# arielmission-space/PAOS

Measured on AMD Instinct MI355X. Metric: wavefronts/sec (4096^2 c128, 20-surface chain) + achieved HBM GB/s, higher is better.
Workload: dtype c128 (f64); 1 GPU; SYN20 20-surface chain (SURVEY 8d: 43 2-D FFTs per wavefront as the reference runs it), 4096x4096 fp64, walked 512-wavelength sweep, 32 wavefronts/GPU/step, PSFs stay in HBM; separable pass programs + ptp identities ([24] passes/wavefront, parity 1e-15..2e-14 vs oracle); grid=4096, batch_per_gpu=32, parallelism=wavefront-sharded x1, transport=none (single process), ranks_seen=1, launcher=none

## Files before the change

include/paos_hip.h:

```cpp
#ifndef PAOS_HIP_H
#define PAOS_HIP_H

#ifdef __cplusplus
extern "C" {
#endif

typedef struct paos_ctx paos_ctx;

enum { PAOS_OK = 0, PAOS_EINVAL = 1, PAOS_EHIP = 2, PAOS_EUNSUPPORTED = 3 };
enum { PAOS_F64 = 0, PAOS_F32 = 1 };
enum { PAOS_SHAPE_ELLIPSE = 0, PAOS_SHAPE_RECT = 1 };
enum { PAOS_KERNEL_PASS_ROWS = 0, PAOS_KERNEL_PASS_COLS = 1, PAOS_KERNEL_PASS_ANY = 2 };
enum { PAOS_PW_SIGN = 1, PAOS_PW_QPHASE_CENTRED = 2, PAOS_PW_QPHASE_NATURAL = 3, PAOS_PW_SCALE = 4,
       PAOS_PW_MASK = 5 };
enum { PAOS_PWF_MUL2PI = 1,
       PAOS_PWF_X_ONLY = 2, PAOS_PWF_Y_ONLY = 4 };
enum { PAOS_MAX_PW = 6 };
enum { PAOS_NORM_SLOTS = 64 };
enum { PAOS_WHAT_FIELD = 0, PAOS_WHAT_AMPLITUDE = 1, PAOS_WHAT_PHASE = 2, PAOS_WHAT_INTENSITY = 3 };

enum { PAOS_PHASE_STRIDE = 5 };
enum { PAOS_APERTURE_STRIDE = 8 };
enum { PAOS_ZERNIKE_HEAD = 8 };

typedef struct { int kind, flags, block; } paos_pw_op;
typedef struct {
  int axis;
  int fft1, fft2;
  int n_pre, n_mid, n_post;
  paos_pw_op pre[PAOS_MAX_PW], mid[PAOS_MAX_PW], post[PAOS_MAX_PW];
} paos_pass;

typedef struct {
  const double* live_rows;
  int rows_stale;
  int final_intensity;
  int* power_ticket;
  const double* live_cols;
} paos_program_opts;

int paos_ctx_create(int device, int n, int batch, int precision, paos_ctx** out);
int paos_ctx_destroy(paos_ctx* ctx);
const char* paos_last_error(const paos_ctx* ctx);
int paos_sync(paos_ctx* ctx);
const char* paos_build_info(void);
const char* paos_source_hash(void);
void* paos_stream(paos_ctx* ctx);

int paos_profile_begin(paos_ctx* ctx, int kernel_kind, int max_launches);
int paos_profile_end(paos_ctx* ctx, int* launches, double* total_ms);
int paos_profile_end_split(paos_ctx* ctx, int* launches, double* total_ms, int* pruned_launches, double* pruned_ms);
int paos_profile_end_launches(paos_ctx* ctx, int capacity, double* ms_out, int* tag_out, int* count);
int paos_profile_planned_bytes(paos_ctx* ctx, int capacity, double* bytes_out, int* count);
int paos_profile_line_transforms(paos_ctx* ctx, int capacity, double* lines_out, int* count);

int paos_fill(paos_ctx* ctx, double re, double im);
int paos_start(paos_ctx* ctx, double re, double im, int shape, const double* aperture, const double* stop);
int paos_start_rows(paos_ctx* ctx, double re, double im, int shape, const double* aperture, const double* stop,
                    const double* write_rows);
int paos_zero_outside_rows(paos_ctx* ctx, const double* live_rows);
int paos_start_box(paos_ctx* ctx, double re, double im, int shape, const double* aperture, const double* stop,
                   const double* write_rows, const double* write_cols);
int paos_zero_outside_box(paos_ctx* ctx, const double* live_rows, const double* live_cols);
int paos_import(paos_ctx* ctx, int item, const void* host_c128);
int paos_export(paos_ctx* ctx, int item, int what, void* host_out);

int paos_psf_keep(paos_ctx* ctx);
int paos_psf_keep_power(paos_ctx* ctx, int* ticket);
int paos_psf_fetch(paos_ctx* ctx, int item, double* host_out);
int paos_host_alloc(unsigned long long bytes, void** out);
int paos_host_free(void* p);
int paos_export_pinned(paos_ctx* ctx, int item, int what, void* pinned_out);

int paos_aperture(paos_ctx* ctx, int shape, const double* params);
int paos_aperture_render(paos_ctx* ctx, int shape, const double* params1, double* host_mask);
int paos_make_stop(paos_ctx* ctx, const double* enable);
int paos_stop_scale_last_power(paos_ctx* ctx, const double* enable);
int paos_stop_defer_last_power(paos_ctx* ctx, const double* enable);
int paos_norm2(paos_ctx* ctx, double* host_out);
int paos_norm2_enqueue(paos_ctx* ctx, int* ticket);
int paos_norm2_enqueue_rows(paos_ctx* ctx, const double* live_rows, int* ticket);
int paos_norm2_enqueue_rows_like(paos_ctx* ctx, const double* live_rows, const double* same_as, int* ticket);
int paos_norm2_enqueue_box(paos_ctx* ctx, const double* live_rows, const double* live_cols, const double* same_as, int* ticket);
int paos_norm2_fetch(paos_ctx* ctx, int ticket, double* host_out);
int paos_norm2_release(paos_ctx* ctx, int ticket);
int paos_psf_metrics(paos_ctx* ctx, int nr, const double* radii_px, double cx_px, double cy_px,
                     double* host_out);
int paos_phase(paos_ctx* ctx, const double* params, int mul2pi);
int paos_phase_map(paos_ctx* ctx, int item, const double* host_wfe, double wl);
int paos_phase_map_items(paos_ctx* ctx, const double* host_wfe, unsigned long long key, int n_items, const double* items,
                         const double* wl);
int paos_psd_screen(paos_ctx* ctx, const double* host_noise, const double* host_rough, const double* params,
                    unsigned long long key, double* host_out);
int paos_ptp(paos_ctx* ctx, const double* params);
int paos_stw(paos_ctx* ctx, const double* params, int inverse);
int paos_wts(paos_ctx* ctx, const double* params, int inverse);
int paos_run_passes(paos_ctx* ctx, const paos_pass* passes, int n_passes, const double* blocks,
                    int n_blocks);
int paos_copy_yardstick(paos_ctx* ctx, int reps, double* ms_per_launch, double* bytes_per_launch);
int paos_record_set_stats(paos_ctx* ctx, unsigned long long* found, unsigned long long* rendered);
int paos_ctx_set_pruning(paos_ctx* ctx, int on);
int paos_run_passes_live(paos_ctx* ctx, const paos_pass* passes, int n_passes, const double* blocks,
                         int n_blocks, const double* live_rows);
int paos_run_program(paos_ctx* ctx, const paos_pass* passes, int n_passes, const double* blocks, int n_blocks,
                     const paos_program_opts* opts);
int paos_zernike(paos_ctx* ctx, int nmax, int kdim, const double* table, const double* params,
                 int param_stride, double* host_wfe);
int paos_zernike_like(paos_ctx* ctx, int nmax, int kdim, const double* table, const double* params,
                      int param_stride, const double* same_as, double* host_wfe);


int paos_pupil_aperture(paos_ctx* ctx, int shape, const double* params);
int paos_pupil_upload(paos_ctx* ctx, int item, const double* host_weights);
int paos_zernike_gram(paos_ctx* ctx, int nmax, int kdim, const double* table, const double* params,
                      int param_stride, int K, const double* poly, int use_pupil, double* host_out);
int paos_zernike_pupil(paos_ctx* ctx, int nmax, int kdim, const double* table, const double* params,
                       int param_stride, double* host_wfe);

enum { PAOS_DETECTOR_GEOM = 6 };
enum { PAOS_DETECTOR_ITEM = 3 };
enum { PAOS_DETECTOR_SCRATCH_MIB = 512 };
int paos_detector_begin(paos_ctx* ctx, const double* geom);
int paos_detector_add(paos_ctx* ctx, const double* per_item);
int paos_detector_images(paos_ctx* ctx, const double* per_item, double* host_out);
int paos_detector_fetch(paos_ctx* ctx, double* host_out);
enum { PAOS_DETECTOR_PLACED_ITEM = 5 };
int paos_detector_add_placed(paos_ctx* ctx, const double* per_item);
int paos_detector_images_placed(paos_ctx* ctx, const double* per_item, double* host_out);

#ifdef __cplusplus
}
#endif
#endif
```

paos_amd/_lib.py:

```python
import ctypes
import os
import threading
import weakref

import numpy as np

_HERE = os.path.dirname(os.path.abspath(__file__))
LIB_PATH = os.environ.get("PAOS_LIB") or os.path.join(_HERE, "libpaoship.so")

PAOS_F64, PAOS_F32 = 0, 1
SHAPE_ELLIPSE, SHAPE_RECT = 0, 1
WHAT_FIELD, WHAT_AMPLITUDE, WHAT_PHASE, WHAT_INTENSITY = 0, 1, 2, 3
KERNEL_PASS_ROWS, KERNEL_PASS_COLS, KERNEL_PASS_ANY = 0, 1, 2
PW_SIGN, PW_QPHASE_CENTRED, PW_QPHASE_NATURAL, PW_SCALE, PW_MASK = 1, 2, 3, 4, 5
PWF_MUL2PI = 1
PWF_X_ONLY, PWF_Y_ONLY = 2, 4
MAX_PW = 6
NORM_SLOTS = 64


class PwOp(ctypes.Structure):
    _fields_ = [("kind", ctypes.c_int), ("flags", ctypes.c_int), ("block", ctypes.c_int)]


class ProgramOpts(ctypes.Structure):
    _fields_ = [("live_rows", ctypes.POINTER(ctypes.c_double)), ("rows_stale", ctypes.c_int),
                ("final_intensity", ctypes.c_int), ("power_ticket", ctypes.POINTER(ctypes.c_int)),
                ("live_cols", ctypes.POINTER(ctypes.c_double))]


class Pass(ctypes.Structure):
    _fields_ = [("axis", ctypes.c_int), ("fft1", ctypes.c_int), ("fft2", ctypes.c_int),
                ("n_pre", ctypes.c_int), ("n_mid", ctypes.c_int), ("n_post", ctypes.c_int),
                ("pre", PwOp * MAX_PW), ("mid", PwOp * MAX_PW), ("post", PwOp * MAX_PW)]

PHASE_STRIDE = 5
APERTURE_STRIDE = 8
ZERNIKE_HEAD = 8

_c_ctx = ctypes.c_void_p
_dbl_p = ctypes.POINTER(ctypes.c_double)
SYMBOLS = {
    "paos_ctx_create": (ctypes.c_int, [ctypes.c_int, ctypes.c_int, ctypes.c_int, ctypes.c_int, ctypes.POINTER(_c_ctx)]),
    "paos_ctx_destroy": (ctypes.c_int, [_c_ctx]),
    "paos_last_error": (ctypes.c_char_p, [_c_ctx]),
    "paos_sync": (ctypes.c_int, [_c_ctx]),
    "paos_build_info": (ctypes.c_char_p, []),
    "paos_stream": (ctypes.c_void_p, [_c_ctx]),
    "paos_profile_begin": (ctypes.c_int, [_c_ctx, ctypes.c_int, ctypes.c_int]),
    "paos_profile_end": (ctypes.c_int, [_c_ctx, ctypes.POINTER(ctypes.c_int), _dbl_p]),
    "paos_profile_end_split": (ctypes.c_int, [_c_ctx, ctypes.POINTER(ctypes.c_int), _dbl_p, ctypes.POINTER(ctypes.c_int), _dbl_p]),
    "paos_source_hash": (ctypes.c_char_p, []),
    "paos_profile_planned_bytes": (ctypes.c_int, [_c_ctx, ctypes.c_int, _dbl_p, ctypes.POINTER(ctypes.c_int)]),
    "paos_profile_line_transforms": (ctypes.c_int, [_c_ctx, ctypes.c_int, _dbl_p, ctypes.POINTER(ctypes.c_int)]),
    "paos_profile_end_launches": (ctypes.c_int, [_c_ctx, ctypes.c_int, _dbl_p, ctypes.POINTER(ctypes.c_int),
                                                 ctypes.POINTER(ctypes.c_int)]),
    "paos_fill": (ctypes.c_int, [_c_ctx, ctypes.c_double, ctypes.c_double]),
    "paos_import": (ctypes.c_int, [_c_ctx, ctypes.c_int, ctypes.c_void_p]),
    "paos_export": (ctypes.c_int, [_c_ctx, ctypes.c_int, ctypes.c_int, ctypes.c_void_p]),
    "paos_aperture": (ctypes.c_int, [_c_ctx, ctypes.c_int, _dbl_p]),
    "paos_aperture_render": (ctypes.c_int, [_c_ctx, ctypes.c_int, _dbl_p, _dbl_p]),
    "paos_make_stop": (ctypes.c_int, [_c_ctx, _dbl_p]),
    "paos_stop_scale_last_power": (ctypes.c_int, [_c_ctx, _dbl_p]),
    "paos_stop_defer_last_power": (ctypes.c_int, [_c_ctx, _dbl_p]),
    "paos_norm2": (ctypes.c_int, [_c_ctx, _dbl_p]),
    "paos_norm2_enqueue": (ctypes.c_int, [_c_ctx, ctypes.POINTER(ctypes.c_int)]),
    "paos_norm2_fetch": (ctypes.c_int, [_c_ctx, ctypes.c_int, _dbl_p]),
    "paos_norm2_release": (ctypes.c_int, [_c_ctx, ctypes.c_int]),
    "paos_psf_metrics": (ctypes.c_int, [_c_ctx, ctypes.c_int, _dbl_p, ctypes.c_double, ctypes.c_double, _dbl_p]),
    "paos_phase": (ctypes.c_int, [_c_ctx, _dbl_p, ctypes.c_int]),
    "paos_phase_map": (ctypes.c_int, [_c_ctx, ctypes.c_int, _dbl_p, ctypes.c_double]),
    "paos_ptp": (ctypes.c_int, [_c_ctx, _dbl_p]),
    "paos_stw": (ctypes.c_int, [_c_ctx, _dbl_p, ctypes.c_int]),
    "paos_wts": (ctypes.c_int, [_c_ctx, _dbl_p, ctypes.c_int]),
    "paos_run_passes": (ctypes.c_int, [_c_ctx, ctypes.POINTER(Pass), ctypes.c_int, _dbl_p, ctypes.c_int]),
    "paos_copy_yardstick": (ctypes.c_int, [_c_ctx, ctypes.c_int, _dbl_p, _dbl_p]),
    "paos_record_set_stats": (ctypes.c_int, [_c_ctx, ctypes.POINTER(ctypes.c_ulonglong), ctypes.POINTER(ctypes.c_ulonglong)]),
    "paos_ctx_set_pruning": (ctypes.c_int, [_c_ctx, ctypes.c_int]),
    "paos_run_passes_live": (ctypes.c_int, [_c_ctx, ctypes.POINTER(Pass), ctypes.c_int, _dbl_p, ctypes.c_int, _dbl_p]),
    "paos_zernike": (ctypes.c_int, [_c_ctx, ctypes.c_int, ctypes.c_int, _dbl_p, _dbl_p, ctypes.c_int, _dbl_p]),
    "paos_psf_keep": (ctypes.c_int, [_c_ctx]),
    "paos_psf_keep_power": (ctypes.c_int, [_c_ctx, ctypes.POINTER(ctypes.c_int)]),
    "paos_psf_fetch": (ctypes.c_int, [_c_ctx, ctypes.c_int, _dbl_p]),
    "paos_host_alloc": (ctypes.c_int, [ctypes.c_ulonglong, ctypes.POINTER(ctypes.c_void_p)]),
    "paos_host_free": (ctypes.c_int, [ctypes.c_void_p]),
    "paos_export_pinned": (ctypes.c_int, [_c_ctx, ctypes.c_int, ctypes.c_int, ctypes.c_void_p]),
    "paos_start": (ctypes.c_int, [_c_ctx, ctypes.c_double, ctypes.c_double, ctypes.c_int, _dbl_p, _dbl_p]),
    "paos_pupil_aperture": (ctypes.c_int, [_c_ctx, ctypes.c_int, _dbl_p]),
    "paos_pupil_upload": (ctypes.c_int, [_c_ctx, ctypes.c_int, _dbl_p]),
    "paos_zernike_like": (ctypes.c_int, [_c_ctx, ctypes.c_int, ctypes.c_int, _dbl_p, _dbl_p, ctypes.c_int, _dbl_p, _dbl_p]),
    "paos_zernike_gram": (ctypes.c_int, [_c_ctx, ctypes.c_int, ctypes.c_int, _dbl_p, _dbl_p, ctypes.c_int,
                                         ctypes.c_int, _dbl_p, ctypes.c_int, _dbl_p]),
    "paos_zernike_pupil": (ctypes.c_int, [_c_ctx, ctypes.c_int, ctypes.c_int, _dbl_p, _dbl_p, ctypes.c_int, _dbl_p]),
    "paos_start_rows": (ctypes.c_int, [_c_ctx, ctypes.c_double, ctypes.c_double, ctypes.c_int, _dbl_p, _dbl_p, _dbl_p]),
    "paos_zero_outside_rows": (ctypes.c_int, [_c_ctx, _dbl_p]),
    "paos_phase_map_items": (ctypes.c_int, [_c_ctx, _dbl_p, ctypes.c_ulonglong, ctypes.c_int, _dbl_p, _dbl_p]),
    "paos_psd_screen": (ctypes.c_int, [_c_ctx, _dbl_p, _dbl_p, _dbl_p, ctypes.c_ulonglong, _dbl_p]),
    "paos_start_box": (ctypes.c_int, [_c_ctx, ctypes.c_double, ctypes.c_double, ctypes.c_int, _dbl_p, _dbl_p, _dbl_p, _dbl_p]),
    "paos_zero_outside_box": (ctypes.c_int, [_c_ctx, _dbl_p, _dbl_p]),
    "paos_norm2_enqueue_box": (ctypes.c_int, [_c_ctx, _dbl_p, _dbl_p, _dbl_p, ctypes.POINTER(ctypes.c_int)]),
    "paos_norm2_enqueue_rows": (ctypes.c_int, [_c_ctx, _dbl_p, ctypes.POINTER(ctypes.c_int)]),
    "paos_norm2_enqueue_rows_like": (ctypes.c_int, [_c_ctx, _dbl_p, _dbl_p, ctypes.POINTER(ctypes.c_int)]),
    "paos_run_program": (ctypes.c_int, [_c_ctx, ctypes.POINTER(Pass), ctypes.c_int, _dbl_p, ctypes.c_int,
                                        ctypes.POINTER(ProgramOpts)]),
    "paos_detector_begin": (ctypes.c_int, [_c_ctx, _dbl_p]),
    "paos_detector_add": (ctypes.c_int, [_c_ctx, _dbl_p]),
    "paos_detector_images": (ctypes.c_int, [_c_ctx, _dbl_p, _dbl_p]),
    "paos_detector_fetch": (ctypes.c_int, [_c_ctx, _dbl_p]),
    "paos_detector_add_placed": (ctypes.c_int, [_c_ctx, _dbl_p]),
    "paos_detector_images_placed": (ctypes.c_int, [_c_ctx, _dbl_p, _dbl_p]),
}

_lib = None


class PaosHipError(RuntimeError):
    pass


def load():
    global _lib
    if _lib is not None:
        return _lib
    if not os.path.exists(LIB_PATH):
        raise PaosHipError(
            f"{LIB_PATH} not found: build it with `make` or "
            "`python -c 'import __graft_entry__ as g; g.build()'` (there is no CPU fallback)"
        )
    lib = ctypes.CDLL(LIB_PATH)
    if os.environ.get("PAOS_LIB"):
        import sys

        print(f"paos_amd: using the library variant {LIB_PATH} (PAOS_LIB)", file=sys.stderr)
    for name, (res, args) in SYMBOLS.items():
        fn = getattr(lib, name)
        fn.restype = res
        fn.argtypes = args
    _lib = lib
    return lib


def _dptr(arr):
    return arr.ctypes.data_as(_dbl_p)


def as_blocks(blocks, batch, stride):
    arr = np.ascontiguousarray(blocks, dtype=np.float64)
    if arr.shape != (batch, stride):
        raise ValueError(f"expected parameter blocks of shape {(batch, stride)}, got {arr.shape}")
    return arr


PINNED_MIN_BYTES = 4 << 20
PINNED_MAX_BYTES = 32 << 20
PINNED_LIVE_BYTES = int(os.environ.get("PAOS_PINNED_BYTES", 8 << 30))
PINNED_POOL_BYTES = 2 << 30
_pin_lock = threading.Lock()
_pin_free = {}
_pin_live = 0
_pin_pooled = 0
# ... 293 lines not shown

    def norm2_release(self, ticket):
        if hasattr(ticket, "release"):
            return ticket.release()
        self._check(self._lib.paos_norm2_release(self._ctx, int(ticket)), "paos_norm2_release")

    def psf_metrics(self, radii_px=(), centre=None):
        r = np.ascontiguousarray(radii_px, dtype=np.float64).reshape(-1)
        cxp, cyp = (self.n / 2, self.n / 2) if centre is None else centre
        out = np.empty((self.batch, 4 + r.size), dtype=np.float64)
        self._check(self._lib.paos_psf_metrics(self._ctx, int(r.size), _dptr(r) if r.size else None,
                                               float(cxp), float(cyp), _dptr(out)), "paos_psf_metrics")
        res = []
        for row in out:
            p = row[0]
            res.append({"power": p, "centroid": (row[1] / p, row[2] / p) if p > 0 else (np.nan, np.nan),
                        "peak": row[3], "encircled": row[4:].copy()})
        return res

    def phase(self, blocks, mul2pi):
        b = as_blocks(blocks, self.batch, PHASE_STRIDE)
        self._check(self._lib.paos_phase(self._ctx, _dptr(b), int(bool(mul2pi))), "paos_phase")

    def phase_map(self, item, wfe, wl):
        w = np.ascontiguousarray(wfe, dtype=np.float64)
        if w.shape != (self.n, self.n):
            raise ValueError(f"phase map must have shape {(self.n, self.n)}")
        self._check(self._lib.paos_phase_map(self._ctx, int(item), _dptr(w), float(wl)), "paos_phase_map")

    def phase_map_items(self, wfe, items, wls, key=0):
        w = None
        if wfe is not None:
            w = np.ascontiguousarray(wfe, dtype=np.float64)
            if w.shape != (self.n, self.n):
                raise ValueError(f"phase map must have shape {(self.n, self.n)}")
        it = np.ascontiguousarray(items, dtype=np.float64).reshape(-1)
        wl = np.ascontiguousarray(wls, dtype=np.float64).reshape(-1)
        if it.size != wl.size or it.size < 1:
            raise ValueError("one wavelength per listed item is required")
        self._check(self._lib.paos_phase_map_items(self._ctx, _dptr(w) if w is not None else None, int(key) & 0xFFFFFFFFFFFFFFFF,
                                                   int(it.size), _dptr(it), _dptr(wl)), "paos_phase_map_items")

    def psd_screen(self, noise, rough, params, key, want_map=False):
        nz = np.ascontiguousarray(noise, dtype=np.float64)
        if nz.shape != (self.n, self.n):
            raise ValueError(f"the noise must have shape {(self.n, self.n)}")
        rg = None
        if rough is not None:
            rg = np.ascontiguousarray(rough, dtype=np.float64)
            if rg.shape != (self.n, self.n):
                raise ValueError(f"the roughness draw must have shape {(self.n, self.n)}")
        pr = np.ascontiguousarray(params, dtype=np.float64).reshape(-1)
        if pr.size != 12:
            raise ValueError("twelve PSD parameters are required")
        out = np.empty((self.n, self.n), dtype=np.float64) if want_map else None
        self._check(self._lib.paos_psd_screen(self._ctx, _dptr(nz), _dptr(rg) if rg is not None else None, _dptr(pr),
                                              int(key) & 0xFFFFFFFFFFFFFFFF, _dptr(out) if out is not None else None), "paos_psd_screen")
        return out

    def ptp(self, blocks):
        b = as_blocks(blocks, self.batch, PHASE_STRIDE)
        self._check(self._lib.paos_ptp(self._ctx, _dptr(b)), "paos_ptp")

    def stw(self, blocks, inverse):
        b = as_blocks(blocks, self.batch, PHASE_STRIDE)
        self._check(self._lib.paos_stw(self._ctx, _dptr(b), int(bool(inverse))), "paos_stw")

    def wts(self, blocks, inverse):
        b = as_blocks(blocks, self.batch, PHASE_STRIDE)
        self._check(self._lib.paos_wts(self._ctx, _dptr(b), int(bool(inverse))), "paos_wts")

    def copy_yardstick(self, reps=10):
        ms, nbytes = ctypes.c_double(0.0), ctypes.c_double(0.0)
        self._check(self._lib.paos_copy_yardstick(self._ctx, int(reps), ctypes.byref(ms), ctypes.byref(nbytes)),
                    "paos_copy_yardstick")
        return ms.value, nbytes.value

    def record_set_stats(self):
        found, rendered = ctypes.c_ulonglong(0), ctypes.c_ulonglong(0)
        self._check(self._lib.paos_record_set_stats(self._ctx, ctypes.byref(found), ctypes.byref(rendered)),
                    "paos_record_set_stats")
        return int(found.value), int(rendered.value)

    def set_pruning(self, on):
        self._check(self._lib.paos_ctx_set_pruning(self._ctx, 1 if on else 0), "paos_ctx_set_pruning")

    def run_passes(self, passes, blocks, live_rows=None, rows_stale=False, final_intensity=False, live_cols=None):
        b = np.ascontiguousarray(blocks, dtype=np.float64)
        if b.ndim != 3 or b.shape[1:] != (self.batch, PHASE_STRIDE):
            raise ValueError("blocks must be [n_blocks][batch][5]")
        arr = (Pass * len(passes))()
        for dst, src in zip(arr, passes):
            dst.axis, dst.fft1, dst.fft2 = src["axis"], src.get("fft1", -1), src.get("fft2", -1)
            for name in ("pre", "mid", "post"):
                ops = src.get(name, ())
                if len(ops) > MAX_PW:
                    raise ValueError("too many operators in one pass slot")
                setattr(dst, "n_" + name, len(ops))
                lst = getattr(dst, name)
                for i, (kind, flags, block) in enumerate(ops):
                    lst[i].kind, lst[i].flags, lst[i].block = kind, flags, block
        if rows_stale or final_intensity:
            lr = self._rows(live_rows) if live_rows is not None else None
            lc = self._rows(live_cols) if (live_cols is not None and rows_stale and lr is not None) else None
            ticket = ctypes.c_int(-1)
            opts = ProgramOpts(_dptr(lr) if lr is not None else None, 1 if (rows_stale and lr is not None) else 0,
                               int(final_intensity), ctypes.pointer(ticket), _dptr(lc) if lc is not None else None)
            self._check(self._lib.paos_run_program(self._ctx, arr, len(passes), _dptr(b), b.shape[0], ctypes.byref(opts)),
                        "paos_run_program")
            return ticket.value if final_intensity else None
        if live_rows is not None:
            lr = self._rows(live_rows)
            self._check(self._lib.paos_run_passes_live(self._ctx, arr, len(passes), _dptr(b), b.shape[0], _dptr(lr)),
                        "paos_run_passes_live")
            return None
        self._check(self._lib.paos_run_passes(self._ctx, arr, len(passes), _dptr(b), b.shape[0]),
                    "paos_run_passes")
        return None

    def zernike(self, nmax, kdim, table, blocks, want_wfe=False, pupil=False, same_as=None):
        t = np.ascontiguousarray(table, dtype=np.float64).reshape(-1)
        b = np.ascontiguousarray(blocks, dtype=np.float64)
        if b.ndim != 2 or b.shape[0] != self.batch:
            raise ValueError("zernike blocks must be [batch][stride]")
        out = np.empty((self.n, self.n), dtype=np.float64) if want_wfe else None
        if same_as is not None and not pupil:
            like = np.ascontiguousarray(same_as, dtype=np.float64).reshape(-1)
            if like.size != self.batch:
                raise ValueError("same_as must name an item per item")
            self._check(self._lib.paos_zernike_like(self._ctx, int(nmax), int(kdim), _dptr(t), _dptr(b), int(b.shape[1]),
                                                    _dptr(like), _dptr(out) if want_wfe else None), "paos_zernike_like")
            return out
        fn = self._lib.paos_zernike_pupil if pupil else self._lib.paos_zernike
        self._check(fn(self._ctx, int(nmax), int(kdim), _dptr(t), _dptr(b), int(b.shape[1]),
                       _dptr(out) if want_wfe else None),
                    "paos_zernike_pupil" if pupil else "paos_zernike")
        return out

    def start(self, value, shape, blocks, stop=None, write_rows=None, write_cols=None):
        b = np.ascontiguousarray(blocks, dtype=np.float64)
        if b.shape != (self.batch, APERTURE_STRIDE):
            raise ValueError("aperture blocks must be [batch][8]")
        st = None if stop is None else np.ascontiguousarray(stop, dtype=np.float64)
        if st is not None and st.shape != (self.batch,):
            raise ValueError("stop flags must be [batch]")
        v = complex(value)
        if write_rows is not None and write_cols is not None:
            self._check(self._lib.paos_start_box(self._ctx, v.real, v.imag, int(shape), _dptr(b),
                                                 _dptr(st) if st is not None else None, _dptr(self._rows(write_rows)),
                                                 _dptr(self._rows(write_cols))), "paos_start_box")
            return
        if write_rows is not None:
            self._check(self._lib.paos_start_rows(self._ctx, v.real, v.imag, int(shape), _dptr(b),
                                                  _dptr(st) if st is not None else None, _dptr(self._rows(write_rows))),
                        "paos_start_rows")
            return
        self._check(self._lib.paos_start(self._ctx, v.real, v.imag, int(shape), _dptr(b),
                                         _dptr(st) if st is not None else None), "paos_start")

    def pupil_aperture(self, shape, blocks):
        b = np.ascontiguousarray(blocks, dtype=np.float64)
        if b.shape != (self.batch, APERTURE_STRIDE):
            raise ValueError("aperture blocks must be [batch][8]")
        self._check(self._lib.paos_pupil_aperture(self._ctx, int(shape), _dptr(b)), "paos_pupil_aperture")

    def pupil_upload(self, item, weights):
# ... 20 lines not shown
```

paos_amd/csrc/paos_hip.hip:

```cpp
#ifndef PAOS_PART
#define PAOS_PART -1
#endif
#include "../../include/paos_hip.h"

#include <hip/hip_runtime.h>

#include <cmath>
#include <complex>
#include <cstdio>
#include <cstdlib>
#include <cstring>
#include <mutex>
#include <set>
#include <string>
#include <utility>
#include <type_traits>
#include <vector>

#include "frugal_pass.h"
#if PAOS_PART <= 0
#include "pointwise.h"
#endif

using namespace paos;

#ifndef PAOS_BR
#define PAOS_BR 4
#endif
#ifndef PAOS_PAD_BLOCKS
#define PAOS_PAD_BLOCKS 3
#endif
static constexpr int BR = PAOS_BR;
#ifndef PAOS_F32_BR
#define PAOS_F32_BR 8
#endif
template <typename T, int N>
constexpr int block_rows() { return (sizeof(T) == 4 && N >= 2048) ? PAOS_F32_BR : PAOS_BR; }
#define F32_BR_SWITCH(c, ...)                                                            \
  do {                                                                                   \
    if ((c)->br == PAOS_F32_BR) { constexpr int FBR = PAOS_F32_BR; __VA_ARGS__; }        \
    else { constexpr int FBR = PAOS_BR; __VA_ARGS__; }                                   \
  } while (0)
[[maybe_unused]] static constexpr int kNormSlots = PAOS_NORM_SLOTS;
template <typename T>
struct Lay {
  static constexpr int BC = 2;
};

namespace {

thread_local std::string g_err;

constexpr int kArenaSlabs = 4;
struct Arena {
  double* host = nullptr;
  double* dev = nullptr;
  size_t cap = 0, head = 0;
  int cur = 0;
  int left = -1;
  hipEvent_t fence[kArenaSlabs] = {};
  bool fenced[kArenaSlabs] = {};
  bool used[kArenaSlabs] = {};
};

}

struct paos_ctx {
  int device = 0, n = 0, batch = 0, precision = 0;
  int br = PAOS_BR;
  unsigned pitch = 0, item_stride = 0;
  hipStream_t stream = nullptr;
  double* psf = nullptr;
  double* map_dev = nullptr;
  unsigned long long map_key = 0;
  std::vector<double> start_key;
  double* start_norm2 = nullptr;
  cx<double>* psd_scratch = nullptr;
  int* psd_bad = nullptr;
  double* psf_partial = nullptr;
  int psf_nparts = 0;
  double* pow_partial = nullptr;
  int pow_nparts = 0;
  cx<double>* ptab = nullptr;
  int ptab_slots = 0;
  double* dyn_scale = nullptr;
  bool dyn_pending = false;
  bool norm2_of_field = false;
  int psf_zero_axis = -1;
  std::vector<double> psf_zero_lo, psf_zero_hi;
  bool det_set = false;
  int det_nx = 0, det_ny = 0;
  double det_geom[4] = {};
  double* det_img = nullptr;
  double* det_rows = nullptr;
  size_t det_rows_bytes = 0;
  double* det_out = nullptr;
  size_t det_out_bytes = 0;
  void* bounce[2] = {nullptr, nullptr};
  hipEvent_t bounce_ev[2] = {nullptr, nullptr};
  void* field = nullptr;
  void* tw = nullptr;
  void* staging = nullptr;
  cx<double>* tables = nullptr;
  double* mask = nullptr;
  double* metric_partial = nullptr;
  double* metric_out = nullptr;
  double* metric_host = nullptr;
  struct MaskSet {
    MaskLine* lines = nullptr;
    double* vals = nullptr;
    std::vector<double> key;
    unsigned long long used = 0;
    int line_lo = 0, line_hi = 0;
  };
  static constexpr int kMaskSets = 8;
  MaskSet mask_sets[kMaskSets];
  unsigned long long mask_clock = 0;
  unsigned long long mask_hits = 0, mask_rendered = 0;
  size_t lds_pad = 0;
  int* mask_overflow = nullptr;
  double* partial = nullptr;
  double* norm2 = nullptr;
  double* norm2_host = nullptr;
  bool prune = true;
  int norm_slot = 0;
  bool norm_busy[64] = {};
  int nparts = 0;
  Arena arena;
  std::string err;
  int prof_kind = -1;
  std::vector<hipEvent_t> prof_events;
  std::vector<int> prof_tags;
  int prof_next_tag = 0;
  double prof_next_bytes = 0.0;
  std::vector<double> prof_bytes;
  double prof_next_lines = 0.0;
  std::vector<double> prof_lines;
  size_t prof_used = 0;
};

namespace {

int fail(paos_ctx* c, int code, const std::string& msg) {
  if (c) c->err = msg;
  g_err = msg;
  return code;
}

#define HIPCHK(c, call)                                                                     \
  do {                                                                                      \
    hipError_t e_ = (call);                                                                 \
    if (e_ != hipSuccess)                                                                   \
      return fail((c), PAOS_EHIP,                                                           \
                  std::string(#call) + ": " + hipGetErrorString(e_) + " (" __FILE__ ":" +   \
                      std::to_string(__LINE__) + ")");                                      \
  } while (0)

size_t elem_bytes(const paos_ctx* c) { return c->precision == PAOS_F64 ? 16 : 8; }

int arena_switch(paos_ctx* c) {
  Arena& a = c->arena;
  if (a.left >= 0) {
    HIPCHK(c, hipEventRecord(a.fence[a.left], c->stream));
    a.fenced[a.left] = true;
  }
  a.left = a.cur;
  const int next = (a.cur + 1) % kArenaSlabs;
  if (a.used[next]) {
    if (a.fenced[next]) HIPCHK(c, hipEventSynchronize(a.fence[next]));
    else HIPCHK(c, hipStreamSynchronize(c->stream));
  }
  a.fenced[next] = false;
  a.used[next] = true;
  a.cur = next;
  a.head = 0;
  return PAOS_OK;
}

int arena_reserve(paos_ctx* c, size_t total) {
  Arena& a = c->arena;
  total += 64;
  if (total > a.cap) {
    HIPCHK(c, hipStreamSynchronize(c->stream));
    size_t cap = a.cap;
    while (cap < total) cap *= 2;
    double *h = nullptr, *d = nullptr;
    HIPCHK(c, hipHostMalloc(&h, kArenaSlabs * cap * sizeof(double)));
    if (hipMalloc(&d, kArenaSlabs * cap * sizeof(double)) != hipSuccess) {
      (void)hipHostFree(h);
      return fail(c, PAOS_EHIP, "hipMalloc(arena growth)");
    }
    (void)hipHostFree(a.host);
    (void)hipFree(a.dev);
    a.host = h; a.dev = d; a.cap = cap; a.head = 0; a.cur = 0; a.left = -1;
    for (int k = 0; k < kArenaSlabs; ++k) a.fenced[k] = a.used[k] = false;
    a.used[0] = true;
    return PAOS_OK;
  }
  if (a.head + total > a.cap) return arena_switch(c);
  return PAOS_OK;
}

int arena_push(paos_ctx* c, const double* src, size_t count, const double** dev) {
  Arena& a = c->arena;
  if (count > a.cap) return fail(c, PAOS_EINVAL, "parameter block larger than the arena");
  if (a.head + count > a.cap) {
    int rc = arena_switch(c);
    if (rc) return rc;
  }
  double* h = a.host + (size_t)a.cur * a.cap + a.head;
  double* d = a.dev + (size_t)a.cur * a.cap + a.head;
  std::memcpy(h, src, count * sizeof(double));
  HIPCHK(c, hipMemcpyAsync(d, h, count * sizeof(double), hipMemcpyHostToDevice, c->stream));
  *dev = d;
  a.head += (count + 15) & ~size_t(15);
  return PAOS_OK;
}

constexpr size_t kBounceBytes = size_t(4) << 20;
int copy_to_host(paos_ctx* c, void* host, const void* dev, size_t bytes) {
  if (bytes > kBounceBytes) {
    HIPCHK(c, hipMemcpyAsync(host, dev, bytes, hipMemcpyDeviceToHost, c->stream));
    HIPCHK(c, hipStreamSynchronize(c->stream));
    return PAOS_OK;
  }
  for (int i = 0; i < 2; ++i)
    if (!c->bounce[i]) {
      HIPCHK(c, hipHostMalloc(&c->bounce[i], kBounceBytes));
      HIPCHK(c, hipEventCreateWithFlags(&c->bounce_ev[i], hipEventDisableTiming));
    }
  const size_t chunks = (bytes + kBounceBytes - 1) / kBounceBytes;
  auto len = [&](size_t k) { return k + 1 < chunks ? kBounceBytes : bytes - k * kBounceBytes; };
  for (size_t k = 0; k <= chunks; ++k) {
    if (k < chunks) {
      HIPCHK(c, hipMemcpyAsync(c->bounce[k & 1], (const char*)dev + k * kBounceBytes, len(k), hipMemcpyDeviceToHost, c->stream));
      HIPCHK(c, hipEventRecord(c->bounce_ev[k & 1], c->stream));
    }
    if (k > 0) {
      HIPCHK(c, hipEventSynchronize(c->bounce_ev[(k - 1) & 1]));
      std::memcpy((char*)host + (k - 1) * kBounceBytes, c->bounce[(k - 1) & 1], len(k - 1));
    }
  }
  HIPCHK(c, hipStreamSynchronize(c->stream));
  return PAOS_OK;
}

#if PAOS_PART <= 0
int pw_blocks(const paos_ctx* c) {
  const size_t total = (size_t)c->item_stride;
  size_t b = (total + kPwThreads - 1) / kPwThreads;
  return (int)(b < 2048 ? b : 2048);
}
#endif

template <typename T, int N>
struct FftCfg {
  static constexpr int BC = Lay<T>::BC;
  static constexpr int BR = block_rows<T, N>();
  static constexpr int E = 16;
  static constexpr int ROW_LINES = (N >= 2048) ? PAOS_BR / 2 : PAOS_BR;
  static constexpr int FR_ROW_LINES = (N >= 2048) ? BR / 2 : BR;
  static constexpr int COL_LINES = BC;
  static constexpr int ROW_THREADS = ROW_LINES * N / E, COL_THREADS = COL_LINES * N / E;
  static constexpr int ROW_TILES = (ROW_THREADS >= 128) ? 1 : 128 / ROW_THREADS;
  static constexpr int COL_TILES = (COL_THREADS >= 128) ? 1 : 128 / COL_THREADS;
  static constexpr bool ROW_SPLIT = (size_t)ROW_LINES * ROW_TILES * line_lds_bytes<T, N, false>() > 144 * 1024;
  static constexpr bool COL_SPLIT = (size_t)COL_LINES * COL_TILES * line_lds_bytes<T, N, false>() > 144 * 1024;
  static constexpr int MINW = 1;
};

bool timed_launch_begin(paos_ctx* c, int kind) {
  const bool timed = (c->prof_kind == kind || c->prof_kind == PAOS_KERNEL_PASS_ANY) && (c->prof_used + 2 <= c->prof_events.size());
  return timed && hipEventRecord(c->prof_events[c->prof_used], c->stream) == hipSuccess;
}
hipError_t timed_launch_end(paos_ctx* c, int tag) {
  const hipError_t e = hipEventRecord(c->prof_events[c->prof_used + 1], c->stream);
  if (e != hipSuccess) return e;
// ... 411 lines not shown
  }
}
template <typename T, int N, int AXIS>
int frugal_kpre(paos_ctx* c, const FrugalArgs& a, int kpre, int kmid, int nfft) {
  switch (kpre) {
    case 0: return frugal_kmid<T, N, AXIS, 0>(c, a, kmid, nfft);
    case 1: return frugal_kmid<T, N, AXIS, 1>(c, a, kmid, nfft);
    default: return frugal_kmid<T, N, AXIS, 2>(c, a, kmid, nfft);
  }
}
template <typename T, int N>
int frugal_axis(paos_ctx* c, const FrugalArgs& a, int axis, int kpre, int kmid, int nfft) {
  return axis == 0 ? frugal_kpre<T, N, 0>(c, a, kpre, kmid, nfft) : frugal_kpre<T, N, 1>(c, a, kpre, kmid, nfft);
}

}

#define PAOS_HIDDEN __attribute__((visibility("hidden")))
PAOS_HIDDEN int paos_frugal_d1024(paos_ctx* c, const FrugalArgs& a, int axis, int kpre, int kmid, int nfft);
PAOS_HIDDEN int paos_frugal_d2048(paos_ctx* c, const FrugalArgs& a, int axis, int kpre, int kmid, int nfft);
PAOS_HIDDEN int paos_frugal_d4096(paos_ctx* c, const FrugalArgs& a, int axis, int kpre, int kmid, int nfft);
PAOS_HIDDEN int paos_frugal_f2048(paos_ctx* c, const FrugalArgs& a, int axis, int kpre, int kmid, int nfft);
PAOS_HIDDEN int paos_frugal_f4096(paos_ctx* c, const FrugalArgs& a, int axis, int kpre, int kmid, int nfft);
#if PAOS_PART < 0 || PAOS_PART == 1
int paos_frugal_d1024(paos_ctx* c, const FrugalArgs& a, int axis, int kpre, int kmid, int nfft) {
  return frugal_axis<double, 1024>(c, a, axis, kpre, kmid, nfft);
}
#endif
#if PAOS_PART < 0 || PAOS_PART == 2
int paos_frugal_d2048(paos_ctx* c, const FrugalArgs& a, int axis, int kpre, int kmid, int nfft) {
  return frugal_axis<double, 2048>(c, a, axis, kpre, kmid, nfft);
}
#endif
#if PAOS_PART < 0 || PAOS_PART == 3
int paos_frugal_d4096(paos_ctx* c, const FrugalArgs& a, int axis, int kpre, int kmid, int nfft) {
  return frugal_axis<double, 4096>(c, a, axis, kpre, kmid, nfft);
}
#endif
#if PAOS_PART < 0 || PAOS_PART == 4
int paos_frugal_f2048(paos_ctx* c, const FrugalArgs& a, int axis, int kpre, int kmid, int nfft) {
  return frugal_axis<float, 2048>(c, a, axis, kpre, kmid, nfft);
}
#endif
#if PAOS_PART < 0 || PAOS_PART == 5
int paos_frugal_f4096(paos_ctx* c, const FrugalArgs& a, int axis, int kpre, int kmid, int nfft) {
  return frugal_axis<float, 4096>(c, a, axis, kpre, kmid, nfft);
}
#endif

#if PAOS_PART <= 0
namespace {

__global__ void dyn_scale_set_kernel(double* dyn, const double* norm2, const double* enable, int batch) {
  const int i = blockIdx.x * blockDim.x + threadIdx.x;
  if (i < batch) dyn[i] = (!enable || enable[i] != 0.0) ? 1.0 / sqrt(norm2[i]) : 1.0;
}
__global__ void dyn_scale_reset_kernel(double* dyn, int batch) {
  const int i = blockIdx.x * blockDim.x + threadIdx.x;
  if (i < batch) dyn[i] = 1.0;
}
template <typename T>
__global__ void scale_by_kernel(cx<T>* field, const double* dyn, unsigned item_stride) {
  const int item = blockIdx.y;
  const double s = dyn[item];
  if (s == 1.0) return;
  cx<T>* f = field + (size_t)item * item_stride;
  for (size_t m = (size_t)blockIdx.x * blockDim.x + threadIdx.x; m < item_stride; m += (size_t)gridDim.x * blockDim.x)
    f[m] = {(T)__dmul_rn((double)f[m].x, s), (T)__dmul_rn((double)f[m].y, s)};
}
int settle_scale(paos_ctx* c, bool field_is_overwritten = false) {
  if (!c->dyn_pending) return PAOS_OK;
  if (!field_is_overwritten) {
    const dim3 grid(pw_blocks(c), c->batch), block(kPwThreads);
    if (c->precision == PAOS_F64)
      hipLaunchKernelGGL(scale_by_kernel<double>, grid, block, 0, c->stream, (cx<double>*)c->field, c->dyn_scale, c->item_stride);
    else
      hipLaunchKernelGGL(scale_by_kernel<float>, grid, block, 0, c->stream, (cx<float>*)c->field, c->dyn_scale, c->item_stride);
  }
  hipLaunchKernelGGL(dyn_scale_reset_kernel, dim3((c->batch + 255) / 256), dim3(256), 0, c->stream, c->dyn_scale, c->batch);
  HIPCHK(c, hipGetLastError());
  c->dyn_pending = false;
  return PAOS_OK;
}
#define SETTLE_SCALE(c) do { if (c) { (c)->norm2_of_field = false; if ((c)->dyn_pending) { int rc_ = settle_scale(c); if (rc_) return rc_; } } } while (0)
#define DROP_SCALE(c) do { if (c) { (c)->norm2_of_field = false; if ((c)->dyn_pending) { int rc_ = settle_scale(c, true); if (rc_) return rc_; } } } while (0)


bool frugal_sizes(const paos_ctx* c) {
  return use_frugal() && c->n >= (c->precision == PAOS_F64 ? 1024 : 2048);
}

int ensure_mask_store(paos_ctx* c) {
  if (!c->mask_overflow) {
    HIPCHK(c, hipMalloc(&c->mask_overflow, sizeof(int)));
    HIPCHK(c, hipMemsetAsync(c->mask_overflow, 0, sizeof(int), c->stream));
  }
  return PAOS_OK;
}

int mask_render_mode() {
  const char* e = getenv("PAOS_MASK_SCAN");
  if (e && e[0] == '1') return 0;
  const char* pe = getenv("PAOS_MASK_PAIRS");
  return (pe && pe[0] == '0') ? 1 : ((pe && pe[0] == '1') ? 2 : 3);
}
bool mask_rect_blocks() {
  const char* e = getenv("PAOS_MASK_RECT_BLOCKS");
  return !(e && e[0] == '0');
}

int assign_mask_set(paos_ctx* c, const paos_pass& p, LoweredPass& lp, const double* blocks) {
  std::vector<double> key;
  key.reserve((size_t)2 * c->batch * FP_STRIDE + c->batch + 3);
  key.push_back((double)p.axis);
  key.push_back((double)(mask_render_mode() + (mask_rect_blocks() ? 0 : 8)));
  const double* ap = blocks + (size_t)lp.mask_block * c->batch * FP_STRIDE;
  key.insert(key.end(), ap, ap + (size_t)2 * c->batch * FP_STRIDE);
  key.insert(key.end(), lp.mask_shared.begin(), lp.mask_shared.end());
  int hit = -1, victim = 0;
  for (int k = 0; k < paos_ctx::kMaskSets; ++k) {
    const paos_ctx::MaskSet& ms = c->mask_sets[k];
    if (!ms.key.empty() && ms.key.size() == key.size() && !std::memcmp(ms.key.data(), key.data(), key.size() * sizeof(double))) hit = k;
    if (ms.used < c->mask_sets[victim].used) victim = k;
  }
  const int k = hit >= 0 ? hit : victim;
  paos_ctx::MaskSet& ms = c->mask_sets[k];
  if (!ms.lines) {
    for (paos_ctx::MaskSet& m2 : c->mask_sets) {
      if (m2.lines) continue;
      HIPCHK(c, hipMalloc(&m2.lines, (size_t)c->batch * c->n * sizeof(MaskLine)));
      HIPCHK(c, hipMalloc(&m2.vals, (size_t)c->batch * c->n * 2 * kMaskW * sizeof(double)));
    }
  }
  ms.used = ++c->mask_clock;
  lp.mask_set = k;
  lp.mask_render = hit < 0;
  lp.mask_shapes = 0;
  for (int it = 0; it < c->batch; ++it) {
    const double* a1 = ap + (size_t)it * FP_STRIDE;
    const double* a2 = a1 + (size_t)c->batch * FP_STRIDE;
    if (a1[0] != 0.0 && (it >= (int)lp.mask_shared.size() || lp.mask_shared[it] == 0.0)) lp.mask_shapes |= (int)a2[3] == 0 ? 1 : 2;
  }
  if (hit < 0) { ms.key = std::move(key); ++c->mask_rendered; } else ++c->mask_hits;
  for (int it = 0; it < c->batch; ++it) {
    if (lp.mask_rep[it] < 0) continue;
    FrugalSlot& sl = lp.mask_slot == 0 ? lp.items[it].pre : lp.items[it].mid;
    sl.lines = ms.lines + (size_t)lp.mask_rep[it] * c->n;
    sl.vals = ms.vals + (size_t)lp.mask_rep[it] * c->n * 2 * kMaskW;
  }
  return PAOS_OK;
}

void forget_mask_sets(paos_ctx* c) {
  for (auto& ms : c->mask_sets) ms.key.clear();
}

MaskJob mask_job(paos_ctx* c, const paos_pass& p, const LoweredPass& lp, const double* ap, const double* dshared) {
  const paos_ctx::MaskSet& ms = c->mask_sets[lp.mask_set];
  const int line0 = lp.mask_lo, line_end = lp.mask_hi > lp.mask_lo ? lp.mask_hi : c->n;
  return MaskJob{ap, dshared, ms.lines, ms.vals, p.axis, line0, line_end, lp.mask_shapes};
}
int launch_mask_jobs(paos_ctx* c, MaskJobs& jobs, int count) {
  jobs.batch_stride = c->batch * (int)FP_STRIDE; jobs.param_stride = (int)FP_STRIDE; jobs.n = c->n; jobs.overflow = c->mask_overflow;
  {
    const int mode = mask_render_mode();
    jobs.windows = mode != 0 ? 1 : 0;
    jobs.pairs = mode >= 2 ? mode - 1 : 0;
    jobs.rect_blocks = mask_rect_blocks() ? 1 : 0;
// ... 216 lines not shown
  int rc;
  if ((rc = check_ops(c, p.pre, p.n_pre, n_blocks))) return rc;
  if ((rc = check_ops(c, p.mid, p.n_mid, n_blocks))) return rc;
  if ((rc = check_ops(c, p.post, p.n_post, n_blocks))) return rc;
  if (p.fft1 >= n_blocks || p.fft2 >= n_blocks) return fail(c, PAOS_EINVAL, "transform control block out of range");
  {
    const paos_pw_op* lists3[3] = {p.pre, p.mid, p.post};
    const int counts3[3] = {p.n_pre, p.n_mid, p.n_post};
    int nmask = 0;
    for (int l = 0; l < 3; ++l)
      for (int o = 0; o < counts3[l]; ++o)
        if (lists3[l][o].kind == PAOS_PW_MASK) {
          if (++nmask > 1) return fail(c, PAOS_EINVAL, "one aperture operator per pass");
          if (!c->mask) HIPCHK(c, hipMalloc(&c->mask, (size_t)c->batch * c->item_stride * sizeof(double)));
          const double* ap = dblocks + (size_t)lists3[l][o].block * c->batch * FP_STRIDE;
          const dim3 grid(pw_blocks(c), c->batch), block(kPwThreads);
          const double* ap2 = ap + (size_t)c->batch * FP_STRIDE;
          if (c->precision == PAOS_F64) {
            hipLaunchKernelGGL((aperture_kernel<double, BR, Lay<double>::BC, 0>), grid, block, 0, c->stream, (cx<double>*)nullptr, ap, ap2, FP_STRIDE, c->n, c->pitch, c->item_stride, c->mask, 1);
            hipLaunchKernelGGL((aperture_kernel<double, BR, Lay<double>::BC, 1>), grid, block, 0, c->stream, (cx<double>*)nullptr, ap, ap2, FP_STRIDE, c->n, c->pitch, c->item_stride, c->mask, 1);
          } else {
            F32_BR_SWITCH(c, hipLaunchKernelGGL((aperture_kernel<float, FBR, Lay<float>::BC, 0>), grid, block, 0, c->stream, (cx<float>*)nullptr, ap, ap2, FP_STRIDE, c->n, c->pitch, c->item_stride, c->mask, 1));
            F32_BR_SWITCH(c, hipLaunchKernelGGL((aperture_kernel<float, FBR, Lay<float>::BC, 1>), grid, block, 0, c->stream, (cx<float>*)nullptr, ap, ap2, FP_STRIDE, c->n, c->pitch, c->item_stride, c->mask, 1));
          }
          HIPCHK(c, hipGetLastError());
        }
  }
  PassArgs a{};
  a.field = c->field; a.tw = c->tw; a.blocks = dblocks; a.tables = c->tables; a.mask = c->mask; a.batch = c->batch;
  a.fft1 = p.fft1; a.fft2 = p.fft2; a.n_pre = p.n_pre; a.n_mid = p.n_mid; a.n_post = p.n_post;
  static_assert(sizeof(PwOp) == sizeof(paos_pw_op), "ABI op layout");
  std::memcpy(a.pre, p.pre, sizeof(a.pre));
  std::memcpy(a.mid, p.mid, sizeof(a.mid));
  std::memcpy(a.post, p.post, sizeof(a.post));
  PwOp* lists[3] = {a.pre, a.mid, a.post};
  const int counts[3] = {a.n_pre, a.n_mid, a.n_post};
  int feat = 0;
  for (int l = 0; l < 3; ++l)
    for (int o = 0; o < PAOS_MAX_PW; ++o) {
      lists[l][o].flags &= (1 << kTableShift) - 1;
      const int t = table_of_op[l * PAOS_MAX_PW + o];
      if (t >= 0) { lists[l][o].flags |= (t + 1) << kTableShift; feat = 3; }
      if (o < counts[l] && lists[l][o].kind == PWK_MASK) feat = 3;
    }
  a.pitch = c->pitch; a.item_stride = c->item_stride;
  if (p.axis == 0 || p.axis == 1)
    return c->precision == PAOS_F64 ? pass_t<double>(c, p.axis, a, feat) : pass_t<float>(c, p.axis, a, feat);
  if (p.axis != -1) return fail(c, PAOS_EINVAL, "pass axis must be 0, 1 or -1");
  if (p.fft1 >= 0 || p.fft2 >= 0 || p.n_mid || p.n_post)
    return fail(c, PAOS_EINVAL, "a transform-free pass carries its operators in the pre list");
  const dim3 grid(pw_blocks(c), c->batch), block(kPwThreads);
  if (c->precision == PAOS_F64)
    hipLaunchKernelGGL((pointwise_kernel<double, BR, Lay<double>::BC>), grid, block, 0, c->stream, a, c->n);
  else
    F32_BR_SWITCH(c, hipLaunchKernelGGL((pointwise_kernel<float, FBR, Lay<float>::BC>), grid, block, 0, c->stream, a, c->n));
  HIPCHK(c, hipGetLastError());
  return PAOS_OK;
}

bool use_pruning() {
  static const bool on = [] { const char* e = getenv("PAOS_NO_PRUNE"); return !(e && e[0] == '1'); }();
  return on;
}

int zero_outside_rows(paos_ctx* c, const double* live_rows);
int zero_outside_box(paos_ctx* c, const double* live_rows, const double* live_cols);
int psf_power_ticket(paos_ctx* c, const double* partial, int nparts, int* ticket, const double* source = nullptr);
int psf_keep_power_impl(paos_ctx* c, int* ticket);

int run_passes_impl(paos_ctx* c, const paos_pass* passes, int n_passes, const double* blocks, int n_blocks,
                    const double* entry_rows, bool entry_stale, int* final_ticket, int final_mode, const double* entry_cols);

int run_passes(paos_ctx* c, const paos_pass* passes, int n_passes, const double* blocks, int n_blocks,
               const double* entry_rows = nullptr, bool entry_stale = false, int* final_ticket = nullptr, int final_mode = 1,
               const double* entry_cols = nullptr) {
  const int rc = run_passes_impl(c, passes, n_passes, blocks, n_blocks, entry_rows, entry_stale, final_ticket, final_mode, entry_cols);
  if (rc != PAOS_OK && c) forget_mask_sets(c);
  return rc;
}

int run_passes_impl(paos_ctx* c, const paos_pass* passes, int n_passes, const double* blocks, int n_blocks,
                    const double* entry_rows, bool entry_stale, int* final_ticket, int final_mode, const double* entry_cols) {
  if (!c || !passes || !blocks || n_passes < 0 || n_blocks < 1) return fail(c, PAOS_EINVAL, "bad pass program");
  c->norm2_of_field = false;
  if (final_ticket && c->norm_busy[next_norm_slot(c)])
    return fail(c, PAOS_EINVAL, "64 power reductions outstanding: fetch earlier tickets (paos_norm2_fetch) first");
  for (int i = 0; i < n_passes; ++i) {
    const paos_pw_op* lists[3] = {passes[i].pre, passes[i].mid, passes[i].post};
    const int counts[3] = {passes[i].n_pre, passes[i].n_mid, passes[i].n_post};
    for (int l = 0; l < 3; ++l)
      for (int o = 0; o < counts[l] && o < PAOS_MAX_PW; ++o) {
        const paos_pw_op& op = lists[l][o];
        if (op.kind != PAOS_PW_QPHASE_CENTRED && op.kind != PAOS_PW_QPHASE_NATURAL) continue;
        if (op.block < 0 || op.block >= n_blocks) return fail(c, PAOS_EINVAL, "operator block index out of range");
        for (int it = 0; it < c->batch; ++it) {
          const double* p = blocks + ((size_t)op.block * c->batch + it) * FP_STRIDE;
          if (p[FP_ENABLE] == 0.0) continue;
          const double hx = 0.5 * c->n * p[FP_SX], hy = 0.5 * c->n * p[FP_SY];
          double arg = std::fabs(p[FP_COEF]) * (hx * hx + hy * hy);
          if (op.flags & PAOS_PWF_MUL2PI) arg *= 6.283185307179586;
          if (!(arg < kMaxPhaseArg))
            return fail(c, PAOS_EUNSUPPORTED, "quadratic phase exceeds 1e12 rad at the grid corner (or is not finite)");
        }
      }
  }
  const double* dblocks = nullptr;
  const size_t per_pass = (((size_t)c->batch * sizeof(FrugalItem) / sizeof(double) + 15) & ~size_t(15)) +
                          (((size_t)c->batch + 15) & ~size_t(15)) + 16;
  int rc = arena_reserve(c, (size_t)n_blocks * c->batch * FP_STRIDE + 16 + (size_t)n_passes * per_pass);
  if (rc) return rc;
  rc = arena_push(c, blocks, (size_t)n_blocks * c->batch * FP_STRIDE, &dblocks);
  if (rc) return rc;
  std::vector<LoweredPass> low(n_passes);
  bool all_frugal = !use_tables() && frugal_sizes(c) && n_passes > 0;
  if (!use_tables() && frugal_sizes(c)) {
    if ((rc = ensure_mask_store(c))) return rc;
    for (int q = 0; q < n_passes; ++q) {
      LoweredPass& lp = low[q];
      lp.ok = lower_frugal(c, passes[q], blocks, lp.items, lp.kpre, lp.kmid, lp.nfft, lp.mask_block, lp.mask_slot, lp.mask_shared,
                           lp.mask_rep);
      if (lp.ok && lp.mask_block >= 0 && (rc = assign_mask_set(c, passes[q], lp, blocks))) return rc;
      all_frugal = all_frugal && lp.ok;
    }
  }
  if (c->dyn_pending) {
    bool ride = n_passes > 0 && low[0].ok;
    if (ride)
      for (const FrugalItem& fi : low[0].items) ride = ride && fi.active != 0.0;
    if (!ride && (rc = settle_scale(c))) return rc;
  }
  const bool pruned = all_frugal && use_pruning() && c->prune;
  if (pruned) plan_pruning(c, passes, n_passes, blocks, low, entry_rows, entry_stale, entry_cols);
  {
    for (int q = 0; q < n_passes; ++q) {
      LoweredPass& lp = low[q];
      if (!lp.ok || lp.mask_block < 0) continue;
      double lo = (double)c->n, hi = 0.0;
      for (const FrugalItem& fi : lp.items) {
        if (fi.active == 0.0) continue;
        lo = fi.line_lo < lo ? fi.line_lo : lo;
        hi = fi.line_hi > hi ? fi.line_hi : hi;
      }
      const bool window = hi > lo;
      lp.mask_lo = window ? (int)lo : 0;
      lp.mask_hi = window ? (int)hi : c->n;
      paos_ctx::MaskSet& ms = c->mask_sets[lp.mask_set];
      if (!lp.mask_render && !(ms.line_lo <= lp.mask_lo && ms.line_hi >= lp.mask_hi)) {
        lp.mask_render = true;
        --c->mask_hits; ++c->mask_rendered;
      }
      if (lp.mask_render) { ms.line_lo = lp.mask_lo; ms.line_hi = lp.mask_hi; }
    }
  }
  if (entry_stale && entry_rows) {
    bool need = !pruned;
    for (int it = 0; it < c->batch && !need; ++it) {
      bool active = false;
      for (int q = 0; q < n_passes; ++q) active = active || low[q].items[it].active != 0.0;
      need = !active;
    }
    const double* windows[2] = {entry_rows, entry_cols};
    for (int w = 0; w < 2 && !need; ++w)
      for (int it = 0; windows[w] && it < c->batch && !need; ++it) {
        const int br = c->br, l = ((int)windows[w][2 * it] / br) * br;
        int h = (((int)windows[w][2 * it + 1] + br - 1) / br) * br;
        if (h > c->n) h = c->n;
// ... 435 lines not shown
  }
  if (c->arena.host) (void)hipHostFree(c->arena.host);
  if (c->arena.dev) (void)hipFree(c->arena.dev);
  for (int k = 0; k < kArenaSlabs; ++k)
    if (c->arena.fence[k]) (void)hipEventDestroy(c->arena.fence[k]);
  if (c->stream) (void)hipStreamDestroy(c->stream);
  delete c;
  return PAOS_OK;
}

static int check_mask_overflow(paos_ctx* c) {
  if (!c->mask_overflow) return PAOS_OK;
  int n = 0;
  HIPCHK(c, hipMemcpy(&n, c->mask_overflow, sizeof(int), hipMemcpyDeviceToHost));
  if (n != 0) {
    (void)hipMemset(c->mask_overflow, 0, sizeof(int));
    for (auto& ms : c->mask_sets) ms.key.clear();
    return fail(c, PAOS_EUNSUPPORTED, "aperture line records overflowed (partial run longer than kMaskW): results are invalid");
  }
  return PAOS_OK;
}

int paos_sync(paos_ctx* c) {
  if (c) (void)hipSetDevice(c->device);
  if (!c) return fail(c, PAOS_EINVAL, "null context");
  HIPCHK(c, hipStreamSynchronize(c->stream));
  return check_mask_overflow(c);
}

int paos_fill(paos_ctx* c, double re, double im) {
  DROP_SCALE(c);
  if (c) (void)hipSetDevice(c->device);
  if (!c) return fail(c, PAOS_EINVAL, "null context");
  const size_t total = (size_t)c->item_stride * c->batch;
  if (c->precision == PAOS_F64)
    hipLaunchKernelGGL(fill_kernel<double>, dim3(2048), dim3(kPwThreads), 0, c->stream,
                       (cx<double>*)c->field, total, re, im);
  else
    hipLaunchKernelGGL(fill_kernel<float>, dim3(2048), dim3(kPwThreads), 0, c->stream,
                       (cx<float>*)c->field, total, (float)re, (float)im);
  HIPCHK(c, hipGetLastError());
  return PAOS_OK;
}

static int check_rows(paos_ctx* c, const double* rows) {
  for (int i = 0; i < c->batch; ++i)
    if (!(rows[2 * i] >= 0.0) || !(rows[2 * i + 1] <= (double)c->n) || !(rows[2 * i] <= rows[2 * i + 1]))
      return fail(c, PAOS_EINVAL, "row range must satisfy 0 <= lo <= hi <= n");
  return PAOS_OK;
}

static std::vector<double> rounded_cols(const paos_ctx* c, const double* cols) {
  std::vector<double> out((size_t)2 * c->batch);
  for (int i = 0; i < c->batch; ++i) {
    int l = (int)cols[2 * i], h = (int)cols[2 * i + 1];
    l = l < 0 ? 0 : (l / c->br) * c->br;
    h = ((h + c->br - 1) / c->br) * c->br;
    if (h > c->n) h = c->n;
    out[2 * i] = l; out[2 * i + 1] = h;
  }
  return out;
}

static int start_impl(paos_ctx* c, double re, double im, int shape, const double* aperture, const double* stop,
                      const double* write_rows, const double* write_cols = nullptr) {
  if (c) (void)hipSetDevice(c->device);
  if (!c || !aperture) return fail(c, PAOS_EINVAL, "null argument");
  if (shape != PAOS_SHAPE_ELLIPSE && shape != PAOS_SHAPE_RECT) return fail(c, PAOS_EINVAL, "unknown aperture shape");
  std::vector<double> flags(c->batch, 0.0);
  bool any_stop = false;
  if (stop)
    for (int i = 0; i < c->batch; ++i) { flags[i] = stop[i] != 0.0 ? 1.0 : 0.0; any_stop |= flags[i] != 0.0; }
  std::vector<double> power_of(c->batch), compute(c->batch);
  for (int i = 0; i < c->batch; ++i) {
    int rep = i;
    for (int j = 0; j < i; ++j)
      if (flags[j] != 0.0 && !std::memcmp(aperture + (size_t)j * AP_STRIDE, aperture + (size_t)i * AP_STRIDE, AP_STRIDE * sizeof(double))) { rep = j; break; }
    power_of[i] = (double)rep;
    compute[i] = (flags[i] != 0.0 && rep == i) ? 1.0 : 0.0;
  }
  const double *dp = nullptr, *ds = nullptr, *dcompute = nullptr, *dpower_of = nullptr;
  int rc;
  if ((rc = arena_push(c, aperture, (size_t)c->batch * AP_STRIDE, &dp))) return rc;
  if ((rc = arena_push(c, flags.data(), flags.size(), &ds))) return rc;
  if ((rc = arena_push(c, compute.data(), compute.size(), &dcompute))) return rc;
  if ((rc = arena_push(c, power_of.data(), power_of.size(), &dpower_of))) return rc;
  const double* drows = nullptr;
  if (write_rows) {
    if ((rc = check_rows(c, write_rows))) return rc;
    if ((rc = arena_push(c, write_rows, (size_t)2 * c->batch, &drows))) return rc;
  }
  const double* dcols = nullptr;
  if (write_cols) {
    if (!write_rows) return fail(c, PAOS_EINVAL, "a column window needs a row window");
    if ((rc = check_rows(c, write_cols))) return rc;
    const std::vector<double> wc = rounded_cols(c, write_cols);
    if ((rc = arena_push(c, wc.data(), wc.size(), &dcols))) return rc;
  }
  static const bool share_start = [] { const char* e = getenv("PAOS_SHARE_START"); return !(e && e[0] == '0'); }();
  std::vector<double> goff(c->batch, 0.0), glen(c->batch, 0.0), members;
  {
    std::vector<int> lead(c->batch);
    for (int i = 0; i < c->batch; ++i) {
      lead[i] = i;
      if (!share_start) continue;
      for (int j = 0; j < i; ++j)
        if (lead[j] == j && flags[j] == flags[i] &&
            !std::memcmp(aperture + (size_t)j * AP_STRIDE, aperture + (size_t)i * AP_STRIDE, AP_STRIDE * sizeof(double)) &&
            (!write_rows || !std::memcmp(write_rows + 2 * j, write_rows + 2 * i, 2 * sizeof(double))) &&
            (!write_cols || !std::memcmp(write_cols + 2 * j, write_cols + 2 * i, 2 * sizeof(double)))) { lead[i] = j; break; }
    }
    for (int i = 0; i < c->batch; ++i) {
      if (lead[i] != i) continue;
      goff[i] = (double)members.size();
      for (int j = i; j < c->batch; ++j)
        if (lead[j] == i) members.push_back((double)j);
      glen[i] = (double)members.size() - goff[i];
    }
  }
  const double *dgoff = nullptr, *dglen = nullptr, *dmembers = nullptr;
  if ((rc = arena_push(c, goff.data(), goff.size(), &dgoff))) return rc;
  if ((rc = arena_push(c, glen.data(), glen.size(), &dglen))) return rc;
  if ((rc = arena_push(c, members.data(), members.size(), &dmembers))) return rc;
  const dim3 block(kPwThreads);
  bool power_found = false;
  if (any_stop) {
    static const bool memo = [] { const char* e = getenv("PAOS_START_POWER_MEMO"); return !(e && e[0] == '0'); }();
    std::vector<double> key;
    key.reserve(3 + (size_t)c->batch * (AP_STRIDE + 1));
    key.push_back((double)shape); key.push_back(re); key.push_back(im);
    key.insert(key.end(), aperture, aperture + (size_t)c->batch * AP_STRIDE);
    key.insert(key.end(), flags.begin(), flags.end());
    power_found = memo && c->start_norm2 && key.size() == c->start_key.size() &&
                  !std::memcmp(key.data(), c->start_key.data(), key.size() * sizeof(double));
    if (power_found) {
      HIPCHK(c, hipMemcpyAsync(c->norm2, c->start_norm2, (size_t)c->batch * sizeof(double), hipMemcpyDeviceToDevice, c->stream));
    } else {
      c->start_key.clear();
      if (memo) c->start_key = std::move(key);
    }
  }
#define START_LAUNCH(T, BRV, S)                                                                         \
  do {                                                                                                  \
    if (any_stop && !power_found) {                                                                     \
      hipLaunchKernelGGL((start_power_kernel<T, BRV, Lay<T>::BC, S>), dim3(c->nparts, c->batch), block, 0, \
                         c->stream, dp, c->n, c->pitch, c->item_stride, re, im, c->partial, dcompute);  \
      hipLaunchKernelGGL(norm2_final_kernel, dim3(c->batch), block, 0, c->stream, c->partial, c->norm2,   \
                         c->nparts, ds, 1, dpower_of);                                                  \
    }                                                                                                   \
    hipLaunchKernelGGL((start_write_kernel<T, BRV, Lay<T>::BC, S>), dim3(pw_blocks(c), c->batch), block, 0, \
                       c->stream, (cx<T>*)c->field, dp, c->n, c->pitch, c->item_stride, re, im,          \
                       (const double*)c->norm2, ds, drows, dgoff, dglen, dmembers, dcols);              \
  } while (0)
  if (c->precision == PAOS_F64) {
    if (shape == PAOS_SHAPE_ELLIPSE) START_LAUNCH(double, BR, 0); else START_LAUNCH(double, BR, 1);
  } else {
    if (shape == PAOS_SHAPE_ELLIPSE) F32_BR_SWITCH(c, START_LAUNCH(float, FBR, 0)); else F32_BR_SWITCH(c, START_LAUNCH(float, FBR, 1));
  }
#undef START_LAUNCH
  HIPCHK(c, hipGetLastError());
  if (any_stop && !power_found && !c->start_key.empty()) {
    if (!c->start_norm2) HIPCHK(c, hipMalloc(&c->start_norm2, (size_t)c->batch * sizeof(double)));
    HIPCHK(c, hipMemcpyAsync(c->start_norm2, c->norm2, (size_t)c->batch * sizeof(double), hipMemcpyDeviceToDevice, c->stream));
  }
  return PAOS_OK;
}

int paos_start(paos_ctx* c, double re, double im, int shape, const double* aperture, const double* stop) {
  DROP_SCALE(c);
  return start_impl(c, re, im, shape, aperture, stop, nullptr);
}

int paos_start_rows(paos_ctx* c, double re, double im, int shape, const double* aperture, const double* stop,
                    const double* write_rows) {
  DROP_SCALE(c);
  return start_impl(c, re, im, shape, aperture, stop, write_rows);
}

int paos_start_box(paos_ctx* c, double re, double im, int shape, const double* aperture, const double* stop,
                   const double* write_rows, const double* write_cols) {
  DROP_SCALE(c);
  return start_impl(c, re, im, shape, aperture, stop, write_rows, write_cols);
}

int paos_zero_outside_box(paos_ctx* c, const double* live_rows, const double* live_cols) {
  SETTLE_SCALE(c);
  if (c) (void)hipSetDevice(c->device);
  if (!c || !live_rows) return fail(c, PAOS_EINVAL, "null argument");
  int rc = check_rows(c, live_rows);
  if (rc) return rc;
  if (live_cols && (rc = check_rows(c, live_cols))) return rc;
  return zero_outside_box(c, live_rows, live_cols);
}

int paos_zero_outside_rows(paos_ctx* c, const double* live_rows) {
  SETTLE_SCALE(c);
  if (c) (void)hipSetDevice(c->device);
  if (!c || !live_rows) return fail(c, PAOS_EINVAL, "null argument");
  int rc = check_rows(c, live_rows);
  if (rc) return rc;
  return zero_outside_rows(c, live_rows);
}

int paos_import(paos_ctx* c, int item, const void* host) {
  SETTLE_SCALE(c);
  if (c) (void)hipSetDevice(c->device);
  if (!c || !host || item < 0 || item >= c->batch) return fail(c, PAOS_EINVAL, "bad item or null buffer");
  const size_t bytes = (size_t)c->n * c->n * 16;
  HIPCHK(c, hipMemcpyAsync(c->staging, host, bytes, hipMemcpyHostToDevice, c->stream));
  if (c->precision == PAOS_F64)
    hipLaunchKernelGGL((import_kernel<double, BR, Lay<double>::BC>), dim3(pw_blocks(c)), dim3(kPwThreads), 0, c->stream,
                       (cx<double>*)c->field + (size_t)item * c->item_stride, (const cx<double>*)c->staging,
                       c->n, c->pitch);
  else
    F32_BR_SWITCH(c, hipLaunchKernelGGL((import_kernel<float, FBR, Lay<float>::BC>), dim3(pw_blocks(c)), dim3(kPwThreads), 0, c->stream,
                       (cx<float>*)c->field + (size_t)item * c->item_stride, (const cx<double>*)c->staging,
                       c->n, c->pitch));
  HIPCHK(c, hipGetLastError());
  HIPCHK(c, hipStreamSynchronize(c->stream));
  return PAOS_OK;
}

static int export_impl(paos_ctx* c, int item, int what, void* host_out, bool pinned) {
  if (!c || !host_out || item < 0 || item >= c->batch || what < 0 || what > 3)
    return fail(c, PAOS_EINVAL, "bad item/what or null buffer");
  if (c->precision == PAOS_F64)
    hipLaunchKernelGGL((export_kernel<double, BR, Lay<double>::BC>), dim3(pw_blocks(c)), dim3(kPwThreads), 0, c->stream,
                       (const cx<double>*)c->field + (size_t)item * c->item_stride, (double*)c->staging,
                       c->n, c->pitch, what);
  else
    F32_BR_SWITCH(c, hipLaunchKernelGGL((export_kernel<float, FBR, Lay<float>::BC>), dim3(pw_blocks(c)), dim3(kPwThreads), 0, c->stream,
                       (const cx<float>*)c->field + (size_t)item * c->item_stride, (double*)c->staging,
                       c->n, c->pitch, what));
  HIPCHK(c, hipGetLastError());
  const size_t bytes = (size_t)c->n * c->n * (what == PAOS_WHAT_FIELD ? 16 : 8);
  if (pinned) {
    HIPCHK(c, hipMemcpyAsync(host_out, c->staging, bytes, hipMemcpyDeviceToHost, c->stream));
    HIPCHK(c, hipStreamSynchronize(c->stream));
  } else {
    int rc = copy_to_host(c, host_out, c->staging, bytes);
    if (rc) return rc;
  }
  return check_mask_overflow(c);
}

int paos_export(paos_ctx* c, int item, int what, void* host_out) {
  SETTLE_SCALE(c);
  if (c) (void)hipSetDevice(c->device);
  return export_impl(c, item, what, host_out, false);
// ... 260 lines not shown
  }
  return PAOS_OK;
}

int zero_outside_box(paos_ctx* c, const double* live_rows, const double* live_cols) {
  if (!live_cols) return zero_outside_rows(c, live_rows);
  const double *drows = nullptr, *dcols = nullptr;
  int rc;
  if ((rc = arena_push(c, live_rows, (size_t)2 * c->batch, &drows))) return rc;
  const std::vector<double> lc = rounded_cols(c, live_cols);
  if ((rc = arena_push(c, lc.data(), lc.size(), &dcols))) return rc;
  const dim3 grid(pw_blocks(c), c->batch), block(kPwThreads);
  if (c->precision == PAOS_F64)
    hipLaunchKernelGGL((zero_outside_box_kernel<double, BR, Lay<double>::BC>), grid, block, 0, c->stream, (cx<double>*)c->field, c->n,
                       c->pitch, c->item_stride, drows, dcols);
  else
    F32_BR_SWITCH(c, hipLaunchKernelGGL((zero_outside_box_kernel<float, FBR, Lay<float>::BC>), grid, block, 0, c->stream,
                                        (cx<float>*)c->field, c->n, c->pitch, c->item_stride, drows, dcols));
  HIPCHK(c, hipGetLastError());
  return PAOS_OK;
}

}

extern "C" {

int paos_psf_keep_power(paos_ctx* c, int* ticket) {
  SETTLE_SCALE(c);
  if (c) (void)hipSetDevice(c->device);
  if (!c || !ticket) return fail(c, PAOS_EINVAL, "null argument");
  return psf_keep_power_impl(c, ticket);
}

int paos_run_program(paos_ctx* c, const paos_pass* passes, int n_passes, const double* blocks, int n_blocks,
                     const paos_program_opts* opts) {
  if (c) (void)hipSetDevice(c->device);
  if (!opts) return run_passes(c, passes, n_passes, blocks, n_blocks);
  if (c && opts->live_rows) {
    int rc = check_rows(c, opts->live_rows);
    if (rc) return rc;
  }
  if (opts->final_intensity && !opts->power_ticket) return fail(c, PAOS_EINVAL, "final_intensity needs a place for the power ticket");
  if (opts->final_intensity < 0 || opts->final_intensity > 2) return fail(c, PAOS_EINVAL, "final_intensity: 0, 1 (PSF instead of the field) or 2 (field + its power)");
  const bool stale = opts->live_rows && opts->rows_stale != 0;
  if (c && opts->live_cols && stale) {
    int rc = check_rows(c, opts->live_cols);
    if (rc) return rc;
  }
  return run_passes(c, passes, n_passes, blocks, n_blocks, opts->live_rows, stale,
                    opts->final_intensity ? opts->power_ticket : nullptr, opts->final_intensity == 2 ? 2 : 1,
                    stale ? opts->live_cols : nullptr);
}

static int norm2_enqueue_rows_impl(paos_ctx* c, const double* live_rows, const double* same_as, int* ticket,
                                   const double* live_cols = nullptr) {
  if (c) (void)hipSetDevice(c->device);
  if (!c || !ticket || !live_rows) return fail(c, PAOS_EINVAL, "null argument");
  int rc = check_rows(c, live_rows);
  if (rc) return rc;
  const int slot = next_norm_slot(c);
  if (c->norm_busy[slot])
    return fail(c, PAOS_EINVAL, "64 power reductions outstanding: fetch earlier tickets (paos_norm2_fetch) first");
  const double *drows = nullptr, *dlead = nullptr, *dsame = nullptr, *dcols = nullptr;
  if ((rc = arena_push(c, live_rows, (size_t)2 * c->batch, &drows))) return rc;
  if (live_cols) {
    const std::vector<double> lc = rounded_cols(c, live_cols);
    if ((rc = arena_push(c, lc.data(), lc.size(), &dcols))) return rc;
  }
  if (same_as) {
    std::vector<double> lead(c->batch);
    for (int i = 0; i < c->batch; ++i) {
      const int j = (int)same_as[i];
      if (!(same_as[i] >= 0.0) || j >= c->batch || (double)j != same_as[i] || (int)same_as[j] != j)
        return fail(c, PAOS_EINVAL, "same_as must name an item that stands for itself");
      if (live_rows[2 * i] != live_rows[2 * j] || live_rows[2 * i + 1] != live_rows[2 * j + 1] ||
          (live_cols && (live_cols[2 * i] != live_cols[2 * j] || live_cols[2 * i + 1] != live_cols[2 * j + 1])))
        return fail(c, PAOS_EINVAL, "items that share a sum must share their row (and column) window");
      lead[i] = j == i ? 1.0 : 0.0;
    }
    if ((rc = arena_push(c, lead.data(), lead.size(), &dlead))) return rc;
    if ((rc = arena_push(c, same_as, (size_t)c->batch, &dsame))) return rc;
  }
  const dim3 grid(c->nparts, c->batch), block(kPwThreads);
  if (c->precision == PAOS_F64)
    hipLaunchKernelGGL((norm2_partial_kernel<double, BR, Lay<double>::BC>), grid, block, 0, c->stream,
                       (const cx<double>*)c->field, c->partial, c->n, c->pitch, c->item_stride, dlead, 1, drows, dcols);
  else
    F32_BR_SWITCH(c, hipLaunchKernelGGL((norm2_partial_kernel<float, FBR, Lay<float>::BC>), grid, block, 0, c->stream,
                       (const cx<float>*)c->field, c->partial, c->n, c->pitch, c->item_stride, dlead, 1, drows, dcols));
  HIPCHK(c, hipGetLastError());
  return psf_power_ticket(c, c->partial, c->nparts, ticket, dsame);
}

int paos_norm2_enqueue_box(paos_ctx* c, const double* live_rows, const double* live_cols, const double* same_as, int* ticket) {
  SETTLE_SCALE(c);
  if (c && live_cols) {
    int rc = check_rows(c, live_cols);
    if (rc) return rc;
  }
  return norm2_enqueue_rows_impl(c, live_rows, same_as, ticket, live_cols);
}

int paos_norm2_enqueue_rows(paos_ctx* c, const double* live_rows, int* ticket) {
  SETTLE_SCALE(c);
  return norm2_enqueue_rows_impl(c, live_rows, nullptr, ticket);
}

int paos_norm2_enqueue_rows_like(paos_ctx* c, const double* live_rows, const double* same_as, int* ticket) {
  SETTLE_SCALE(c);
  if (!same_as) return fail(c, PAOS_EINVAL, "null argument");
  return norm2_enqueue_rows_impl(c, live_rows, same_as, ticket);
}

int paos_norm2_fetch(paos_ctx* c, int ticket, double* host_out) {
  if (c) (void)hipSetDevice(c->device);
  if (!c || !host_out || ticket < 0 || ticket >= kNormSlots) return fail(c, PAOS_EINVAL, "bad ticket");
  if (!c->norm_busy[ticket]) return fail(c, PAOS_EINVAL, "ticket is not outstanding (already fetched, or never issued)");
  HIPCHK(c, hipStreamSynchronize(c->stream));
  c->norm_busy[ticket] = false;
  std::memcpy(host_out, c->norm2_host + (size_t)ticket * c->batch, (size_t)c->batch * sizeof(double));
  return check_mask_overflow(c);
}

int paos_norm2_release(paos_ctx* c, int ticket) {
  if (!c || ticket < 0 || ticket >= kNormSlots) return fail(c, PAOS_EINVAL, "bad ticket");
  c->norm_busy[ticket] = false;
  return PAOS_OK;
}

int paos_norm2(paos_ctx* c, double* host_out) {
  SETTLE_SCALE(c);
  if (c) (void)hipSetDevice(c->device);
  if (!c || !host_out) return fail(c, PAOS_EINVAL, "null argument");
  int rc = norm2_launch(c, nullptr);
  if (rc) return rc;
  HIPCHK(c, hipMemcpyAsync(c->norm2_host, c->norm2, (size_t)c->batch * sizeof(double), hipMemcpyDeviceToHost, c->stream));
  HIPCHK(c, hipStreamSynchronize(c->stream));
  std::memcpy(host_out, c->norm2_host, (size_t)c->batch * sizeof(double));
  return PAOS_OK;
}

int paos_phase(paos_ctx* c, const double* params, int mul2pi) {
  SETTLE_SCALE(c);
  if (c) (void)hipSetDevice(c->device);
  if (!c || !params) return fail(c, PAOS_EINVAL, "null argument");
  Program g(c->batch);
  const int par = g.add_block(params, 0, 0, 0, 0, true);
  paos_pass& p = g.add_pass(-1, -1, -1);
  push(p.pre, p.n_pre, PAOS_PW_QPHASE_CENTRED, par, mul2pi ? PAOS_PWF_MUL2PI : 0);
  return run_passes(c, g.passes.data(), 1, g.blocks.data(), 1);
}

int paos_phase_map(paos_ctx* c, int item, const double* host_wfe, double wl) {
  SETTLE_SCALE(c);
  if (c) (void)hipSetDevice(c->device);
  if (!c || !host_wfe || item < 0 || item >= c->batch) return fail(c, PAOS_EINVAL, "bad item or null buffer");
  if (!(wl > 0.0) || !std::isfinite(wl)) return fail(c, PAOS_EINVAL, "wavelength must be positive and finite");
  const size_t count = (size_t)c->n * c->n;
  for (size_t i = 0; i < count; ++i)
    if (!std::isfinite(host_wfe[i])) return fail(c, PAOS_EINVAL, "the phase map holds a non-finite value (fill masked pixels with 0)");
  HIPCHK(c, hipMemcpyAsync(c->staging, host_wfe, count * sizeof(double), hipMemcpyHostToDevice, c->stream));
  if (c->precision == PAOS_F64)
    hipLaunchKernelGGL((phase_map_kernel<double, BR, Lay<double>::BC>), dim3(pw_blocks(c)), dim3(kPwThreads), 0, c->stream,
                       (cx<double>*)c->field + (size_t)item * c->item_stride, (const double*)c->staging, c->n, c->pitch, wl);
  else
    F32_BR_SWITCH(c, hipLaunchKernelGGL((phase_map_kernel<float, FBR, Lay<float>::BC>), dim3(pw_blocks(c)), dim3(kPwThreads), 0, c->stream,
                       (cx<float>*)c->field + (size_t)item * c->item_stride, (const double*)c->staging, c->n, c->pitch, wl));
  HIPCHK(c, hipGetLastError());
  HIPCHK(c, hipStreamSynchronize(c->stream));
  return PAOS_OK;
}

int paos_phase_map_items(paos_ctx* c, const double* host_wfe, unsigned long long key, int n_items, const double* items,
                         const double* wl) {
  SETTLE_SCALE(c);
  if (c) (void)hipSetDevice(c->device);
  if (!c || !items || !wl || n_items < 1 || n_items > c->batch) return fail(c, PAOS_EINVAL, "bad item list or null buffer");
  if (!host_wfe && (key == 0 || key != c->map_key || !c->map_dev)) return fail(c, PAOS_EINVAL, "no host map, and no map kept on the device under this key");
// ... 9 lines not shown
    c->map_key = 0;
    HIPCHK(c, hipMemcpyAsync(c->map_dev, host_wfe, count * sizeof(double), hipMemcpyHostToDevice, c->stream));
    HIPCHK(c, hipStreamSynchronize(c->stream));
    c->map_key = key;
  }
  const double *ditems = nullptr, *dwl = nullptr;
  int rc;
  if ((rc = arena_push(c, items, (size_t)n_items, &ditems))) return rc;
  if ((rc = arena_push(c, wl, (size_t)n_items, &dwl))) return rc;
  const dim3 grid(pw_blocks(c), n_items), block(kPwThreads);
  if (c->precision == PAOS_F64)
    hipLaunchKernelGGL((phase_map_items_kernel<double, BR, Lay<double>::BC>), grid, block, 0, c->stream, (cx<double>*)c->field,
                       c->item_stride, (const double*)c->map_dev, c->n, c->pitch, ditems, dwl);
  else
    F32_BR_SWITCH(c, hipLaunchKernelGGL((phase_map_items_kernel<float, FBR, Lay<float>::BC>), grid, block, 0, c->stream,
                                        (cx<float>*)c->field, c->item_stride, (const double*)c->map_dev, c->n, c->pitch, ditems, dwl));
  HIPCHK(c, hipGetLastError());
  return PAOS_OK;
}

int paos_psd_screen(paos_ctx* c, const double* host_noise, const double* host_rough, const double* params, unsigned long long key,
                    double* host_out) {
  if (c) (void)hipSetDevice(c->device);
  if (!c || !host_noise || !params || key == 0) return fail(c, PAOS_EINVAL, "null argument (or key 0)");
  if (c->precision != PAOS_F64) return fail(c, PAOS_EUNSUPPORTED, "PSD screens are built on complex128 contexts (build the map on the host for fp32 mode)");
  PsdParams p{params[0], params[1], params[2], params[3], params[4], params[5], params[6], params[7], params[8], params[9], params[10], params[11]};
  for (int k = 0; k < 12; ++k)
    if (std::isnan(params[k])) return fail(c, PAOS_EINVAL, "a PSD parameter is NaN");
  const size_t count = (size_t)c->n * c->n;
  if (!c->map_dev) HIPCHK(c, hipMalloc(&c->map_dev, count * sizeof(double)));
  if (!c->psd_scratch) HIPCHK(c, hipMalloc(&c->psd_scratch, (size_t)c->item_stride * sizeof(cx<double>)));
  if (!c->psd_bad) HIPCHK(c, hipMalloc(&c->psd_bad, sizeof(int)));
  c->map_key = 0;
  double* noise = (double*)c->staging;
  double* rough = (host_rough && p.SR != 0.0) ? noise + count : nullptr;
  HIPCHK(c, hipMemcpyAsync(noise, host_noise, count * sizeof(double), hipMemcpyHostToDevice, c->stream));
  if (rough) HIPCHK(c, hipMemcpyAsync(rough, host_rough, count * sizeof(double), hipMemcpyHostToDevice, c->stream));
  HIPCHK(c, hipMemsetAsync(c->psd_bad, 0, sizeof(int), c->stream));
  std::vector<double> hb((size_t)3 * FP_STRIDE, 0.0);
  hb[0 * FP_STRIDE + FP_ENABLE] = 1.0;
  hb[1 * FP_STRIDE + FP_ENABLE] = 1.0; hb[1 * FP_STRIDE + 1] = 1.0;
  hb[2 * FP_STRIDE + FP_ENABLE] = 1.0; hb[2 * FP_STRIDE + 3] = 1.0 / c->n;
  const double* dblocks = nullptr;
  int rc;
  if ((rc = arena_push(c, hb.data(), hb.size(), &dblocks))) return rc;
  const dim3 grid(pw_blocks(c)), block(kPwThreads);
  hipLaunchKernelGGL((psd_load_kernel<BR, Lay<double>::BC>), grid, block, 0, c->stream, c->psd_scratch, (const double*)noise, c->n, c->pitch);
  PassArgs a{};
  a.field = c->psd_scratch; a.tw = c->tw; a.blocks = dblocks; a.tables = nullptr; a.mask = nullptr; a.batch = 1;
  a.fft1 = 0; a.fft2 = -1; a.pitch = c->pitch; a.item_stride = c->item_stride;
  for (int axis = 0; axis < 2; ++axis)
    if ((rc = pass_t<double>(c, axis, a, 0))) return rc;
  hipLaunchKernelGGL((psd_filter_kernel<BR, Lay<double>::BC>), grid, block, 0, c->stream, c->psd_scratch, c->n, c->pitch, p);
  a.fft1 = 1; a.n_mid = 1; a.mid[0] = {PAOS_PW_SCALE, 0, 2};
  for (int axis = 0; axis < 2; ++axis)
    if ((rc = pass_t<double>(c, axis, a, 0))) return rc;
  hipLaunchKernelGGL((psd_finish_kernel<BR, Lay<double>::BC>), grid, block, 0, c->stream, c->map_dev, (const cx<double>*)c->psd_scratch,
                     (const double*)rough, c->n, c->pitch, p, c->psd_bad);
  HIPCHK(c, hipGetLastError());
  int bad = 0;
  HIPCHK(c, hipMemcpyAsync(&bad, c->psd_bad, sizeof(int), hipMemcpyDeviceToHost, c->stream));
  HIPCHK(c, hipStreamSynchronize(c->stream));
  if (bad) return fail(c, PAOS_EINVAL, "the PSD screen holds a non-finite value");
  if (host_out) {
    rc = copy_to_host(c, host_out, c->map_dev, count * sizeof(double));
    if (rc) return rc;
  }
  c->map_key = key;
  return PAOS_OK;
}

int paos_run_passes(paos_ctx* c, const paos_pass* passes, int n_passes, const double* blocks, int n_blocks) {
  if (c) (void)hipSetDevice(c->device);
  return run_passes(c, passes, n_passes, blocks, n_blocks);
}

int paos_record_set_stats(paos_ctx* c, unsigned long long* found, unsigned long long* rendered) {
  if (!c || !found || !rendered) return fail(c, PAOS_EINVAL, "bad record-set request");
  *found = c->mask_hits;
  *rendered = c->mask_rendered;
  return PAOS_OK;
}

int paos_copy_yardstick(paos_ctx* c, int reps, double* ms_per_launch, double* bytes_per_launch) {
  SETTLE_SCALE(c);
  if (c) (void)hipSetDevice(c->device);
  if (!c || !ms_per_launch || !bytes_per_launch || reps < 1) return fail(c, PAOS_EINVAL, "bad yardstick request");
  const size_t total = (size_t)c->item_stride * c->batch;
  const int blocks = (int)((total + kPwThreads - 1) / kPwThreads < 65536 * 4 ? (total + kPwThreads - 1) / kPwThreads : 65536 * 4);
  hipEvent_t e0, e1;
  HIPCHK(c, hipEventCreate(&e0));
  HIPCHK(c, hipEventCreate(&e1));
  auto launch = [&] {
    if (c->precision == PAOS_F64)
      hipLaunchKernelGGL(rmw_copy_kernel<double>, dim3(blocks), dim3(kPwThreads), 0, c->stream, (cx<double>*)c->field, total);
    else
      hipLaunchKernelGGL(rmw_copy_kernel<float>, dim3(blocks), dim3(kPwThreads), 0, c->stream, (cx<float>*)c->field, total);
  };
  launch();
  HIPCHK(c, hipEventRecord(e0, c->stream));
  for (int r = 0; r < reps; ++r) launch();
  HIPCHK(c, hipEventRecord(e1, c->stream));
  HIPCHK(c, hipEventSynchronize(e1));
  float ms = 0.f;
  HIPCHK(c, hipEventElapsedTime(&ms, e0, e1));
  (void)hipEventDestroy(e0);
  (void)hipEventDestroy(e1);
  *ms_per_launch = (double)ms / reps;
  *bytes_per_launch = 2.0 * (double)total * (double)elem_bytes(c);
  return PAOS_OK;
}

int paos_ctx_set_pruning(paos_ctx* c, int on) {
  if (!c) return fail(c, PAOS_EINVAL, "null context");
  c->prune = on != 0;
  return PAOS_OK;
}

int paos_run_passes_live(paos_ctx* c, const paos_pass* passes, int n_passes, const double* blocks, int n_blocks,
                         const double* live_rows) {
  if (c) (void)hipSetDevice(c->device);
  if (c && live_rows)
    for (int i = 0; i < c->batch; ++i)
      if (!(live_rows[2 * i] >= 0.0) || !(live_rows[2 * i + 1] <= (double)c->n) || !(live_rows[2 * i] <= live_rows[2 * i + 1]))
        return fail(c, PAOS_EINVAL, "live row range must satisfy 0 <= lo <= hi <= n");
  return run_passes(c, passes, n_passes, blocks, n_blocks, live_rows);
}

int paos_ptp(paos_ctx* c, const double* params) {
  if (c) (void)hipSetDevice(c->device);
  return fft_op(c, OP_PTP, params, 0);
}
int paos_stw(paos_ctx* c, const double* params, int inverse) {
  if (c) (void)hipSetDevice(c->device);
  return fft_op(c, OP_STW, params, inverse);
}
int paos_wts(paos_ctx* c, const double* params, int inverse) {
  if (c) (void)hipSetDevice(c->device);
  return fft_op(c, OP_WTS, params, inverse);
}

static int zernike_apply(paos_ctx* c, int nmax, int kdim, const double* table, const double* params,
                         int param_stride, double* host_wfe, bool use_pupil, const double* same_as = nullptr) {
  if (!c || !table || !params) return fail(c, PAOS_EINVAL, "null argument");
  if (nmax < 0 || kdim < nmax / 2 + 1 || param_stride < ZP_HEAD + 2 * (nmax + 1) * kdim)
    return fail(c, PAOS_EINVAL, "inconsistent Zernike table dimensions");
  if (use_pupil && !c->mask) return fail(c, PAOS_EINVAL, "no pupil defined (paos_pupil_aperture / paos_pupil_upload)");
  for (int i = 0; i < c->batch; ++i) {
    const double* q = params + (size_t)i * param_stride;
    if (q[ZP_ENABLE] == 0.0) continue;
    if (!(q[ZP_RADIUS] > 0.0)) return fail(c, PAOS_EINVAL, "Zernike radius must be > 0");
    for (int k = ZP_DX; k < param_stride; ++k)
      if (!std::isfinite(q[k])) return fail(c, PAOS_EINVAL, "non-finite Zernike parameter");
  }
  const double *dt = nullptr, *dp = nullptr;
  int rc = arena_push(c, table, (size_t)(nmax + 1) * kdim * 3, &dt);
  if (rc) return rc;
  rc = arena_push(c, params, (size_t)c->batch * param_stride, &dp);
  if (rc) return rc;
  static const bool share_wfe = [] { const char* e = getenv("PAOS_SHARE_WFE"); return !(e && e[0] == '0'); }();
  std::vector<double> goff(c->batch, 0.0), glen(c->batch, 0.0), members;
  {
    std::vector<int> lead(c->batch, -1);
    auto same_map = [&](int a, int b) {
      const double *qa = params + (size_t)a * param_stride, *qb = params + (size_t)b * param_stride;
      for (int k = 0; k < param_stride; ++k)
        if (k != ZP_INV_WL && std::memcmp(qa + k, qb + k, sizeof(double))) return false;
      return true;
    };
    for (int i = 0; i < c->batch; ++i) {
      if (params[(size_t)i * param_stride + ZP_ENABLE] == 0.0) continue;
      lead[i] = i;
      if (share_wfe && !use_pupil)
        for (int j = 0; j < i; ++j)
          if (lead[j] == j && same_map(j, i)) { lead[i] = j; break; }
    }
    for (int i = 0; i < c->batch; ++i) {
      if (lead[i] != i) continue;
      goff[i] = (double)members.size();
      for (int j = i; j < c->batch; ++j)
        if (lead[j] == i) members.push_back((double)j);
      glen[i] = (double)members.size() - goff[i];
    }
    if (members.empty()) members.push_back(0.0);
  }
  const double *dgoff = nullptr, *dglen = nullptr, *dmembers = nullptr, *dtwins = nullptr;
  if ((rc = arena_push(c, goff.data(), goff.size(), &dgoff))) return rc;
  if ((rc = arena_push(c, glen.data(), glen.size(), &dglen))) return rc;
  if ((rc = arena_push(c, members.data(), members.size(), &dmembers))) return rc;
  if (same_as) {
    std::vector<double> twins(c->batch, 0.0);
    bool any = false;
    for (int i = 0; i < c->batch; ++i) {
      if (!(same_as[i] >= 0.0) || same_as[i] >= (double)c->batch || same_as[i] != (double)(int)same_as[i])
        return fail(c, PAOS_EINVAL, "same_as must hold item indices");
      if (glen[i] < 2.0) continue;
      bool all = true;
      for (int g = 0; g < (int)glen[i]; ++g) all = all && same_as[(int)members[(size_t)goff[i] + g]] == same_as[i];
      twins[i] = all ? 1.0 : 0.0;
      any = any || all;
    }
    if (any && (rc = arena_push(c, twins.data(), twins.size(), &dtwins))) return rc;
  }
  const dim3 grid(pw_blocks(c), c->batch), block(kPwThreads);
  double* wfe = host_wfe ? (double*)c->staging : nullptr;
  const double* pupil = use_pupil ? c->mask : nullptr;
  unsigned m_first = 0, m_end = c->item_stride;
  if (!host_wfe) {
    double half = -1.0;
    bool known = true;
    for (int i = 0; i < c->batch; ++i) {
      const double* q = params + (size_t)i * param_stride;
      if (q[ZP_ENABLE] == 0.0) continue;
      const double h = q[ZP_RADIUS] / q[ZP_DY];
      if (!(h >= 0.0) || !std::isfinite(h)) { known = false; break; }
      if (h > half) half = h;
    }
    if (known && half >= 0.0 && half < (double)c->n) {
      int lo = (int)std::floor((double)(c->n / 2) - half) - 2, hi = (int)std::ceil((double)(c->n / 2) + half) + 3;
      lo = lo < 0 ? 0 : (lo / c->br) * c->br;
      hi = hi > c->n ? c->n : ((hi + c->br - 1) / c->br) * c->br;
      if (hi > c->n) hi = c->n;
      m_first = (unsigned)(lo / c->br) * c->pitch;
      m_end = (unsigned)(hi / c->br) * c->pitch;
    }
  }
#define ZK_LAUNCH(T, BRV, NC)                                                                                          \
  hipLaunchKernelGGL((zernike_kernel<T, BRV, Lay<T>::BC, NC>), grid, block, 0, c->stream, (cx<T>*)c->field, dt, dp,   \
                     param_stride, c->n, c->pitch, c->item_stride, nmax, kdim, wfe, pupil, m_first, m_end, dgoff, dglen, \
                     dmembers, dtwins)
  if (c->precision == PAOS_F64) {
    if (nmax <= 8) ZK_LAUNCH(double, BR, 8); else ZK_LAUNCH(double, BR, 0);
  } else {
    if (nmax <= 8) F32_BR_SWITCH(c, ZK_LAUNCH(float, FBR, 8)); else F32_BR_SWITCH(c, ZK_LAUNCH(float, FBR, 0));
  }
#undef ZK_LAUNCH
  HIPCHK(c, hipGetLastError());
  if (host_wfe) return copy_to_host(c, host_wfe, c->staging, (size_t)c->n * c->n * 8);
  return PAOS_OK;
}

int paos_zernike(paos_ctx* c, int nmax, int kdim, const double* table, const double* params,
                 int param_stride, double* host_wfe) {
  SETTLE_SCALE(c);
  if (c) (void)hipSetDevice(c->device);
  return zernike_apply(c, nmax, kdim, table, params, param_stride, host_wfe, false);
}

int paos_zernike_like(paos_ctx* c, int nmax, int kdim, const double* table, const double* params,
                      int param_stride, const double* same_as, double* host_wfe) {
  SETTLE_SCALE(c);
  if (c) (void)hipSetDevice(c->device);
  return zernike_apply(c, nmax, kdim, table, params, param_stride, host_wfe, false, same_as);
}

int paos_zernike_pupil(paos_ctx* c, int nmax, int kdim, const double* table, const double* params,
                       int param_stride, double* host_wfe) {
  SETTLE_SCALE(c);
  if (c) (void)hipSetDevice(c->device);
  return zernike_apply(c, nmax, kdim, table, params, param_stride, host_wfe, true);
}

static int ensure_pupil(paos_ctx* c) {
  if (!c->mask) HIPCHK(c, hipMalloc(&c->mask, (size_t)c->batch * c->item_stride * sizeof(double)));
  return PAOS_OK;
}

int paos_pupil_aperture(paos_ctx* c, int shape, const double* params) {
  if (c) (void)hipSetDevice(c->device);
  if (!c || !params) return fail(c, PAOS_EINVAL, "null argument");
  if (shape != PAOS_SHAPE_ELLIPSE && shape != PAOS_SHAPE_RECT) return fail(c, PAOS_EINVAL, "unknown aperture shape");
  int rc = ensure_pupil(c);
  if (rc) return rc;
  const double* dp = nullptr;
  rc = arena_push(c, params, (size_t)c->batch * AP_STRIDE, &dp);
  if (rc) return rc;
  const dim3 grid(pw_blocks(c), c->batch), block(kPwThreads);
  if (shape == PAOS_SHAPE_ELLIPSE)
    F32_BR_SWITCH(c, hipLaunchKernelGGL((aperture_kernel<double, FBR, Lay<double>::BC, 0>), grid, block, 0, c->stream, (cx<double>*)nullptr,
                       dp, (const double*)nullptr, AP_STRIDE, c->n, c->pitch, c->item_stride, c->mask, 2));
  else
    F32_BR_SWITCH(c, hipLaunchKernelGGL((aperture_kernel<double, FBR, Lay<double>::BC, 1>), grid, block, 0, c->stream, (cx<double>*)nullptr,
                       dp, (const double*)nullptr, AP_STRIDE, c->n, c->pitch, c->item_stride, c->mask, 2));
  HIPCHK(c, hipGetLastError());
  return PAOS_OK;
}

int paos_pupil_upload(paos_ctx* c, int item, const double* host_weights) {
  if (c) (void)hipSetDevice(c->device);
  if (!c || !host_weights) return fail(c, PAOS_EINVAL, "null argument");
  if (item < 0 || item >= c->batch) return fail(c, PAOS_EINVAL, "item out of range");
  int rc = ensure_pupil(c);
  if (rc) return rc;
  HIPCHK(c, hipMemcpyAsync(c->staging, host_weights, (size_t)c->n * c->n * 8, hipMemcpyHostToDevice, c->stream));
  F32_BR_SWITCH(c, hipLaunchKernelGGL((import_weights_kernel<FBR, Lay<double>::BC>), dim3(pw_blocks(c)), dim3(kPwThreads), 0, c->stream,
                     (const double*)c->staging, c->mask + (size_t)item * c->item_stride, c->n, c->pitch, c->item_stride));
  HIPCHK(c, hipGetLastError());
  HIPCHK(c, hipStreamSynchronize(c->stream));
  return PAOS_OK;
}

int paos_zernike_gram(paos_ctx* c, int nmax, int kdim, const double* table, const double* params,
                      int param_stride, int K, const double* poly, int use_pupil, double* host_out) {
  SETTLE_SCALE(c);
  if (c) (void)hipSetDevice(c->device);
  if (!c || !table || !params || !poly || !host_out) return fail(c, PAOS_EINVAL, "null argument");
  if (nmax < 0 || kdim < nmax / 2 + 1 || param_stride < ZP_HEAD)
    return fail(c, PAOS_EINVAL, "inconsistent Zernike table dimensions");
  if (K < 1 || K > kGramMaxK) return fail(c, PAOS_EUNSUPPORTED, "1 <= K <= 64 polynomials");
  if (use_pupil && !c->mask) return fail(c, PAOS_EINVAL, "no pupil defined (paos_pupil_aperture / paos_pupil_upload)");
  for (int i = 0; i < c->batch; ++i) {
    const double* q = params + (size_t)i * param_stride;
    if (q[ZP_ENABLE] == 0.0) continue;
    if (!(q[ZP_RADIUS] > 0.0)) return fail(c, PAOS_EINVAL, "Zernike radius must be > 0");
    for (int k = ZP_DX; k < ZP_HEAD; ++k)
      if (!std::isfinite(q[k])) return fail(c, PAOS_EINVAL, "non-finite Zernike parameter");
  }
  const size_t ncoef = (size_t)(nmax + 1) * kdim;
  std::vector<double> slots(2 * ncoef, -1.0), fac(K);
  for (int j = 0; j < K; ++j) {
    const int am = (int)poly[4 * j], k = (int)poly[4 * j + 1], is_sin = poly[4 * j + 2] != 0.0;
    if (am < 0 || am > nmax || k < 0 || k >= kdim || am + 2 * k > nmax)
      return fail(c, PAOS_EINVAL, "polynomial outside the recurrence table");
    double& slot = slots[2 * ((size_t)am * kdim + k) + (is_sin ? 1 : 0)];
    if (slot >= 0.0) return fail(c, PAOS_EINVAL, "polynomial listed twice");
    slot = (double)j;
    fac[j] = poly[4 * j + 3];
  }
  const double *dt = nullptr, *dp = nullptr, *dslots = nullptr, *dfac = nullptr;
  int rc;
  if ((rc = arena_push(c, table, ncoef * 3, &dt))) return rc;
  if ((rc = arena_push(c, params, (size_t)c->batch * param_stride, &dp))) return rc;
  if ((rc = arena_push(c, slots.data(), slots.size(), &dslots))) return rc;
  if ((rc = arena_push(c, fac.data(), fac.size(), &dfac))) return rc;
// ... 193 lines not shown
```

paos_amd/csrc/pointwise.h:

```cpp
#pragma once
#include "frugal_pass.h"

namespace paos {

template <int BR, int BC>
__device__ __forceinline__ bool layout_unmap(size_t m, int n, unsigned pitch, int& row, int& col) {
  const unsigned brow = (unsigned)(m / pitch), rem = (unsigned)(m % pitch);
  if (rem >= (unsigned)n * BR) return false;
  const unsigned in = rem % (BR * BC);
  row = (int)(brow * BR + in / BC);
  col = (int)((rem / (BR * BC)) * BC + in % BC);
  return true;
}

constexpr int kPwThreads = 256;

template <typename T>
__global__ void fill_kernel(cx<T>* f, size_t total, T re, T im) {
  size_t i = (size_t)blockIdx.x * blockDim.x + threadIdx.x;
  for (; i < total; i += (size_t)gridDim.x * blockDim.x) f[i] = {re, im};
}

template <typename T>
__global__ void rmw_copy_kernel(cx<T>* f, size_t total) {
// ... 464 lines not shown
      hw = a / 2.0;
      hh = b / 2.0;
      xe = fmax(fabs(__dsub_rn(__dmul_rn(hw, ct), __dmul_rn(hh, st))),
                fabs(__dadd_rn(__dmul_rn(hw, ct), __dmul_rn(hh, st))));
      ye = fmax(fabs(__dadd_rn(__dmul_rn(hw, st), __dmul_rn(hh, ct))),
                fabs(__dsub_rn(__dmul_rn(hw, st), __dmul_rn(hh, ct))));
    }
    box = make_box(xc, yc, xe, ye);
  }
  __device__ __forceinline__ double mask(int r, int c) const {
    if (!(c >= box.ixmin && c < box.ixmax && r >= box.iymin && r < box.iymax)) return 0.0;
    if (SHAPE == 0) return ellipse_pixel(c, r, xc, yc, a, b, ct, st, full_disk);
    if (theta == 0.0) {
      const int cxn = subpixel_count_1d(c, xc, hw, subpix);
      const int cyn = subpixel_count_1d(r, yc, hh, subpix);
      return (double)(cxn * cyn) / (double)(subpix * subpix);
    }
    return rect_pixel(c, r, xc, yc, hw, hh, ct, st, subpix);
  }
  __device__ __forceinline__ double weight(double m) const { return obsc ? __dsub_rn(1.0, m) : m; }
};

template <typename T, int BR, int BC, int SHAPE>
__global__ void aperture_kernel(cx<T>* field, const double* params, const double* params2,
                                int param_stride, int n, unsigned pitch, unsigned item_stride,
                                double* mask_out, int weights_out) {
  const int item = blockIdx.y;
  const double* p = params + (size_t)item * param_stride;
  const double* p2 = params2 ? params2 + (size_t)item * param_stride : p + AP_THETA;
  if (p[AP_ENABLE] == 0.0) return;
  if (weights_out == 1 && SHAPE != (int)p2[3]) return;
  ApertureEval<SHAPE> ap;
  ap.init(p, p2);
  cx<T>* f = field ? field + (size_t)item * item_stride : nullptr;
  const size_t total = item_stride;
  size_t m = (size_t)blockIdx.x * blockDim.x + threadIdx.x;
  for (; m < total; m += (size_t)gridDim.x * blockDim.x) {
    int r, c;
    if (!layout_unmap<BR, BC>(m, n, pitch, r, c)) continue;
    const double mask = ap.mask(r, c);
    const double w = ap.weight(mask);
    if (mask_out) {
      if (weights_out) mask_out[(size_t)item * item_stride + m] = w;
      else if (item == 0) mask_out[(size_t)r * n + c] = mask;
      continue;
    }
    if (w == 0.0) {
      f[m] = {(T)0, (T)0};
    } else if (w != 1.0) {
      cx<T> v = f[m];
      v.x = (T)__dmul_rn((double)v.x, w);
      v.y = (T)__dmul_rn((double)v.y, w);
      f[m] = v;
    }
  }
}

template <typename T, int BR, int BC, int SHAPE>
__global__ void start_power_kernel(const double* params, int n, unsigned pitch, unsigned item_stride,
                                   double vre, double vim, double* partial, const double* stop) {
  const int item = blockIdx.y;
  if (stop[item] == 0.0) return;
  __shared__ double sh[kPwThreads / 64];
  const double* p = params + (size_t)item * AP_STRIDE;
  ApertureEval<SHAPE> ap;
  ap.init(p, p + AP_THETA);
  const bool on = p[AP_ENABLE] != 0.0;
  const double v0re = (double)(T)vre, v0im = (double)(T)vim;
  const size_t total = item_stride;
  double acc = 0.0;
  size_t m = (size_t)blockIdx.x * blockDim.x + threadIdx.x;
  for (; m < total; m += (size_t)gridDim.x * blockDim.x) {
    int r, c;
    if (!layout_unmap<BR, BC>(m, n, pitch, r, c)) continue;
    const double w = on ? ap.weight(ap.mask(r, c)) : 1.0;
    const double x = w == 1.0 ? v0re : (w == 0.0 ? 0.0 : (double)(T)__dmul_rn(v0re, w));
    const double y = w == 1.0 ? v0im : (w == 0.0 ? 0.0 : (double)(T)__dmul_rn(v0im, w));
    acc += __dadd_rn(__dmul_rn(x, x), __dmul_rn(y, y));
  }
  const double s = block_sum(acc, sh);
  if (threadIdx.x == 0) partial[(size_t)item * gridDim.x + blockIdx.x] = s;
}

template <typename T, int BR, int BC, int SHAPE>
__global__ void start_write_kernel(cx<T>* field, const double* params, int n, unsigned pitch,
                                   unsigned item_stride, double vre, double vim, const double* norm2,
                                   const double* stop, const double* rows, const double* grp_off,
                                   const double* grp_len, const double* grp_members, const double* cols = nullptr) {
  const int item = blockIdx.y;
  const int glen = (int)grp_len[item];
  if (glen == 0) return;
  const double* members = grp_members + (int)grp_off[item];
  const double* p = params + (size_t)item * AP_STRIDE;
  ApertureEval<SHAPE> ap;
  ap.init(p, p + AP_THETA);
  const bool on = p[AP_ENABLE] != 0.0;
  const bool scaled = stop[item] != 0.0;
  const double s = scaled ? 1.0 / sqrt(norm2[item]) : 1.0;
  const double v0re = (double)(T)vre, v0im = (double)(T)vim;
  size_t total = item_stride, first = 0;
  if (rows) {
    first = (size_t)((int)rows[2 * item] / BR) * pitch;
    total = (size_t)(((int)rows[2 * item + 1] + BR - 1) / BR) * pitch;
    if (total > item_stride) total = item_stride;
  }
  unsigned in_lo = 0, span = pitch;
  if (cols) {
    in_lo = (unsigned)((int)cols[2 * item] / BC) * (BR * BC);
    unsigned h = (unsigned)(((int)cols[2 * item + 1] + BC - 1) / BC) * (BR * BC);
    if (h > (unsigned)n * BR) h = (unsigned)n * BR;
    span = h > in_lo ? h - in_lo : 0;
  }
  const size_t nbr = (total - first) / pitch;
  const size_t work = cols ? nbr * span : total - first;
  for (size_t j = (size_t)blockIdx.x * blockDim.x + threadIdx.x; j < work; j += (size_t)gridDim.x * blockDim.x) {
    const size_t m = cols ? first + (j / span) * pitch + in_lo + (j % span) : first + j;
    int r, c;
    double x = 0.0, y = 0.0;
    if (layout_unmap<BR, BC>(m, n, pitch, r, c)) {
      const double w = on ? ap.weight(ap.mask(r, c)) : 1.0;
      x = w == 1.0 ? v0re : (w == 0.0 ? 0.0 : (double)(T)__dmul_rn(v0re, w));
      y = w == 1.0 ? v0im : (w == 0.0 ? 0.0 : (double)(T)__dmul_rn(v0im, w));
      if (scaled) { x = __dmul_rn(x, s); y = __dmul_rn(y, s); }
    }
    for (int g = 0; g < glen; ++g) field[(size_t)(int)members[g] * item_stride + m] = {(T)x, (T)y};
  }
}

template <typename T, int BR, int BC>
__global__ void zero_outside_box_kernel(cx<T>* field, int n, unsigned pitch, unsigned item_stride, const double* rows,
                                        const double* cols) {
  const int item = blockIdx.y;
  const int rlo = ((int)rows[2 * item] / BR) * BR, rhi = (((int)rows[2 * item + 1] + BR - 1) / BR) * BR;
  const int clo = cols ? ((int)cols[2 * item] / BC) * BC : 0, chi = cols ? (((int)cols[2 * item + 1] + BC - 1) / BC) * BC : n;
  cx<T>* f = field + (size_t)item * item_stride;
  for (size_t m = (size_t)blockIdx.x * blockDim.x + threadIdx.x; m < item_stride; m += (size_t)gridDim.x * blockDim.x) {
    int r, c;
    if (!layout_unmap<BR, BC>(m, n, pitch, r, c)) continue;
    if (r < rlo || r >= rhi || c < clo || c >= chi) f[m] = {(T)0, (T)0};
  }
}

constexpr int kMaskWaves = 4;

struct MaskJob {
  const double* params;
  const double* shared;
  MaskLine* lines;
  double* vals;
  int axis, line0, line_end, shapes;
};
constexpr int kMaskJobs = 8;
struct MaskJobs {
  MaskJob job[kMaskJobs];
  int windows;
  int pairs;
  int rect_blocks;
  int batch_stride;
  int param_stride, n;
  int* overflow;
};

template <int SHAPE>
__device__ void mask_line_render(const MaskJobs& jobs, const MaskJob& jb, int item, int line, int lane) {
  const int n = jobs.n, axis = jb.axis, param_stride = jobs.param_stride;
  int* const overflow = jobs.overflow;
  if (line >= jb.line_end || line >= n) return;
  const double* p = jb.params + (size_t)item * param_stride;
  const double* p2 = jb.params + jobs.batch_stride + (size_t)item * param_stride;
  MaskLine* out = jb.lines + (size_t)item * n + line;
  double* vout = jb.vals + ((size_t)item * n + line) * (2 * kMaskW);
  if (p[AP_ENABLE] == 0.0 || SHAPE != (int)p2[3]) return;
  const double xc = p[AP_XC], yc = p[AP_YC], a = p[AP_A], b = p[AP_B];
  const bool obsc = p2[1] != 0.0;
  const int subpix = (int)p2[2];
  const double w_in = obsc ? 0.0 : 1.0, w_out = obsc ? 1.0 : 0.0;
  double xe, ye, hw = 0.0, hh = 0.0, full_disk = 0.0, lm = 1.0;
  if (SHAPE == 0) {
    xe = sqrt(__dmul_rn(a, a));
    ye = sqrt(__dmul_rn(b, b));
    full_disk = fmin(__dmul_rn(__dmul_rn(3.141592653589793, a), b), 1.0);
  } else {
    hw = a / 2.0; hh = b / 2.0;
    xe = fabs(hw); ye = fabs(hh);
  }
  const ApertureBox box = make_box(xc, yc, xe, ye);
  if (SHAPE == 1) {
    const int c_other = axis == 0 ? subpixel_count_1d(line, yc, hh, subpix) : subpixel_count_1d(line, xc, hw, subpix);
    const bool in_box = axis == 0 ? (line >= box.iymin && line < box.iymax) : (line >= box.ixmin && line < box.ixmax);
    lm = in_box ? (double)c_other / (double)subpix : 0.0;
  }
  int p0 = n, p1 = -1, p2i = -1, p3 = 0;
  const bool line_in_box = axis == 0 ? (line >= box.iymin && line < box.iymax) : (line >= box.ixmin && line < box.ixmax);
  const int scan_lo = line_in_box ? max(0, (axis == 0 ? box.ixmin : box.iymin)) & ~63 : 0;
  const int scan_hi = line_in_box ? min(n, axis == 0 ? box.ixmax : box.iymax) : 0;
  if (SHAPE == 0 && line_in_box && jobs.windows != 0) {
    const double sa = axis == 0 ? a : b, sc = axis == 0 ? b : a;
    const double ca = axis == 0 ? xc : yc, cc = axis == 0 ? yc : xc;
    const double lo_c = __dsub_rn((double)line - 0.5, cc), hi_c = __dsub_rn((double)line + 0.5, cc);
    const double near_c = (lo_c > 0.0 ? lo_c : (hi_c < 0.0 ? -hi_c : 0.0)) / sc;
    const double far_c = fmax(fabs(lo_c), fabs(hi_c)) / sc;
    const double half_long = near_c < 1.0 ? sa * sqrt(1.0 - near_c * near_c) : 0.0;
    const double half_short = far_c < 1.0 ? sa * sqrt(1.0 - far_c * far_c) : 0.0;
    const int box_lo = max(0, axis == 0 ? box.ixmin : box.iymin), box_hi = min(n, axis == 0 ? box.ixmax : box.iymax);
    const int wl0 = max(box_lo, (int)floor(ca - half_long) - 3), wl1 = (int)ceil(ca - half_short) + 3;
    const int wr1 = min(box_hi - 1, (int)ceil(ca + half_long) + 3), wr0 = wr1 - 31;
    const int wr_need = (int)floor(ca + half_short) - 3;
// ... 212 lines not shown
  const ApertureBox box = make_box(xc, yc, fabs(hw), fabs(hh));
  const int line = first + lane;
  const bool valid = line < jb.line_end && line < n;
  const bool in_box = valid && (axis == 0 ? (line >= box.iymin && line < box.iymax) : (line >= box.ixmin && line < box.ixmax));
  const int c_other = axis == 0 ? subpixel_count_1d(line, yc, hh, subpix) : subpixel_count_1d(line, xc, hw, subpix);
  const double lm = in_box ? (double)c_other / (double)subpix : 0.0;
  const unsigned long long in_lines = __ballot(in_box);
  int p0 = n, p1 = -1, p2i = -1, p3 = 0;
  auto weight = [&](int pos) {
    const bool inside = axis == 0 ? (pos >= box.ixmin && pos < box.ixmax) : (pos >= box.iymin && pos < box.iymax);
    return inside ? (double)(axis == 0 ? subpixel_count_1d(pos, xc, hw, subpix) : subpixel_count_1d(pos, yc, hh, subpix)) / (double)subpix : 0.0;
  };
  if (in_lines) {
    const int scan_lo = max(0, (axis == 0 ? box.ixmin : box.iymin)) & ~63, scan_hi = min(n, axis == 0 ? box.ixmax : box.iymax);
    for (int base = scan_lo; base < scan_hi; base += 64) {
      const double w = weight(base + lane);
      const unsigned long long not_out = __ballot(w != 0.0), is_in = __ballot(w == 1.0);
      if (not_out) {
        p0 = min(p0, base + (int)__ffsll((long long)not_out) - 1);
        p3 = max(p3, base + 64 - (int)__clzll((long long)not_out));
      }
      if (is_in) {
        if (p1 < 0) p1 = base + (int)__ffsll((long long)is_in) - 1;
        p2i = base + 64 - (int)__clzll((long long)is_in);
      }
    }
  }
  if (p3 <= p0) { p0 = p1 = p2i = p3 = 0; }
  else if (p1 < 0) { p1 = p2i = p3; }
  if (p1 - p0 > kMaskW || p3 - p2i > kMaskW) {
    if (lane == 0) atomicAdd(jobs.overflow, __popcll(in_lines));
    p0 = p1 = p2i = p3 = 0;
  }
  for (int side = 0; side < 2; ++side) {
    const int lo = side == 0 ? p0 : p2i, hi = side == 0 ? p1 : p3;
    for (int pos = lo + lane; pos < hi; pos += 64) prof[side * kMaskW + pos - lo] = weight(pos);
  }
  __builtin_amdgcn_fence(__ATOMIC_RELEASE, "wavefront");
  __builtin_amdgcn_wave_barrier();
  __builtin_amdgcn_fence(__ATOMIC_ACQUIRE, "wavefront");
  if (valid) {
    MaskLine* out = jb.lines + (size_t)item * n + line;
    if (in_box) *out = {p0, p1, p2i, p3, lm, 0.0}; else *out = {0, 0, 0, 0, lm, 0.0};
  }
  const int len0 = p1 - p0, len1 = p3 - p2i;
  for (unsigned long long todo = in_lines; todo; todo &= todo - 1) {
    const int k = (int)__ffsll((long long)todo) - 1;
    double* vout = jb.vals + ((size_t)item * n + (first + k)) * (2 * kMaskW);
    for (int j = lane; j < len0; j += 64) vout[j] = prof[j];
    for (int j = lane; j < len1; j += 64) vout[kMaskW + j] = prof[kMaskW + j];
  }
}

template <int SHAPE>
__global__ void __launch_bounds__(kMaskWaves * 64) mask_lines_kernel(MaskJobs jobs) {
  const MaskJob& jb = jobs.job[blockIdx.z];
  if (!(jb.shapes & (1 << SHAPE))) return;
  const int item = blockIdx.y;
  if (jb.shared[item] != 0.0) return;
  const int lane = threadIdx.x & 63;
  const int wave = blockIdx.x * (blockDim.x >> 6) + (threadIdx.x >> 6);
  if (SHAPE == 1 && jobs.rect_blocks != 0) {
    __shared__ double prof[kMaskWaves][2 * kMaskW];
    mask_rect_block_render(jobs, jb, item, jb.line0 + 64 * wave, lane, prof[threadIdx.x >> 6]);
    return;
  }
  if (!(SHAPE == 0 && jobs.pairs != 0)) {
    mask_line_render<SHAPE>(jobs, jb, item, jb.line0 + wave, lane);
    return;
  }
  const int per = jobs.pairs >= 2 ? 4 : 2;
  const int first = jb.line0 + per * wave;
  if (first >= jb.line_end || first >= jobs.n) return;
  if (per == 4 && mask_multi_render<4>(jobs, jb, item, first, lane)) return;
  for (int f = first; f < first + per; f += 2) {
    if (mask_multi_render<2>(jobs, jb, item, f, lane)) continue;
    mask_line_render<0>(jobs, jb, item, f, lane);
    mask_line_render<0>(jobs, jb, item, f + 1, lane);
  }
}

enum : int { ZP_ENABLE = 0, ZP_DX, ZP_DY, ZP_RADIUS, ZP_ORIGIN_Y, ZP_COS_OFF, ZP_SIN_OFF, ZP_INV_WL, ZP_HEAD };

template <typename T, int BR, int BC, int NMAXC = 0>
__global__ void zernike_kernel(cx<T>* field, const double* table, const double* params,
                               int param_stride, int n, unsigned pitch, unsigned item_stride,
                               int nmax, int kdim, double* wfe_out, const double* pupil,
                               unsigned m_first, unsigned m_end, const double* grp_off, const double* grp_len,
                               const double* grp_members, const double* grp_twins = nullptr) {
  const int item = blockIdx.y;
  const int glen = (int)grp_len[item];
  if (glen == 0) return;
  const double* members = grp_members + (int)grp_off[item];
  const bool twins = grp_twins && grp_twins[item] != 0.0;
  const double* p = params + (size_t)item * param_stride;
  const double dx = p[ZP_DX], dy = p[ZP_DY], radius = p[ZP_RADIUS];
  const bool origin_y = p[ZP_ORIGIN_Y] != 0.0;
  const double co = p[ZP_COS_OFF], so = p[ZP_SIN_OFF];
  const double* coef_c = p + ZP_HEAD;
  const double* coef_s = coef_c + (size_t)(nmax + 1) * kdim;
  const size_t total = m_end < item_stride ? m_end : item_stride;
  size_t m = (size_t)m_first + (size_t)blockIdx.x * blockDim.x + threadIdx.x;
  for (; m < total; m += (size_t)gridDim.x * blockDim.x) {
    int r, c;
    if (!layout_unmap<BR, BC>(m, n, pitch, r, c)) continue;
    const double x = (double)(c - n / 2) * dx, y = (double)(r - n / 2) * dy;
    const double rr = sqrt(__dadd_rn(__dmul_rn(x, x), __dmul_rn(y, y)));
    const double rho = rr / radius;
    const bool masked = rho > 1.0 || (pupil && pupil[(size_t)item * item_stride + m] == 0.0);
    double wfe = 0.0;
    if (!masked) {
      double c1 = 1.0, s1 = 0.0;
      if (rr > 0.0) {
        c1 = (origin_y ? y : x) / rr;
        s1 = (origin_y ? x : y) / rr;
      }
      const double cr = c1 * co - s1 * so, sr = s1 * co + c1 * so;
      const double xj = 1.0 - 2.0 * rho * rho;
      double rho_pow = 1.0, cm = 1.0, sm = 0.0;
      auto order = [&](int am, int k_end) __attribute__((always_inline)) {
        double pkm1 = 0.0, pk = 1.0;
        for (int k = 0; k <= k_end; ++k) {
          if (k > 0) {
            const double* abc = table + ((size_t)am * kdim + k) * 3;
            const double pn = (abc[0] * xj + abc[1]) * pk - abc[2] * pkm1;
            pkm1 = pk;
            pk = pn;
          }
          const size_t ci = (size_t)am * kdim + k;
          wfe += (rho_pow * pk) * (coef_c[ci] * cm + coef_s[ci] * sm);
        }
        rho_pow *= rho;
        const double cn = cm * cr - sm * sr;
        sm = sm * cr + cm * sr;
        cm = cn;
      };
      if constexpr (NMAXC > 0) {
#pragma unroll
        for (int am = 0; am <= NMAXC; ++am) {
          if (am > nmax) break;
          const int kmax = (nmax - am) / 2;
          double pkm1 = 0.0, pk = 1.0;
#pragma unroll
          for (int k = 0; k <= (NMAXC - am) / 2; ++k) {
            if (k > kmax) break;
            if (k > 0) {
              const double* abc = table + ((size_t)am * kdim + k) * 3;
              const double pn = (abc[0] * xj + abc[1]) * pk - abc[2] * pkm1;
              pkm1 = pk;
              pk = pn;
            }
            const size_t ci = (size_t)am * kdim + k;
            wfe += (rho_pow * pk) * (coef_c[ci] * cm + coef_s[ci] * sm);
          }
          rho_pow *= rho;
          const double cn = cm * cr - sm * sr;
          sm = sm * cr + cm * sr;
          cm = cn;
        }
      } else {
        for (int am = 0; am <= nmax; ++am) order(am, (nmax - am) / 2);
      }
      const double turns = __dmul_rn(6.283185307179586, wfe);
      constexpr int kZernikeGroup = 8;
      cx<double> lead = {0.0, 0.0};
      if (twins) { const cx<T>* fl = field + (size_t)item * item_stride + m; lead = {(double)fl->x, (double)fl->y}; }
      int g = 0;
      for (; g + kZernikeGroup <= glen; g += kZernikeGroup) {
        cx<T>* f4[kZernikeGroup];
        cx<double> v4[kZernikeGroup];
        double iw[kZernikeGroup];
#pragma unroll
        for (int q = 0; q < kZernikeGroup; ++q) {
          const int it = (int)members[g + q];
          f4[q] = field + (size_t)it * item_stride + m;
          iw[q] = params[(size_t)it * param_stride + ZP_INV_WL];
        }
        if (twins) {
#pragma unroll
          for (int q = 0; q < kZernikeGroup; ++q) v4[q] = lead;
        } else {
#pragma unroll
          for (int q = 0; q < kZernikeGroup; ++q) v4[q] = {(double)f4[q]->x, (double)f4[q]->y};
        }
#pragma unroll
        for (int q = 0; q < kZernikeGroup; ++q) {
          double sn, cs;
          sincos_fast(__dmul_rn(turns, iw[q]), &sn, &cs);
          *f4[q] = {(T)__dsub_rn(__dmul_rn(v4[q].x, cs), __dmul_rn(v4[q].y, sn)),
                    (T)__dadd_rn(__dmul_rn(v4[q].x, sn), __dmul_rn(v4[q].y, cs))};
        }
      }
      for (; g < glen; ++g) {
        const int it = (int)members[g];
        const double arg = __dmul_rn(turns, params[(size_t)it * param_stride + ZP_INV_WL]);
        double sn, cs;
        sincos_fast(arg, &sn, &cs);
        cx<T>* f = field + (size_t)it * item_stride;
        const cx<double> v = twins ? lead : cx<double>{(double)f[m].x, (double)f[m].y};
        f[m] = {(T)__dsub_rn(__dmul_rn(v.x, cs), __dmul_rn(v.y, sn)),
                (T)__dadd_rn(__dmul_rn(v.x, sn), __dmul_rn(v.y, cs))};
      }
    }
    if (wfe_out && item == 0) wfe_out[(size_t)r * n + c] = masked ? __longlong_as_double(0x7ff8000000000000LL) : wfe;
  }
}

constexpr int kGramMaxK = 64, kGramPix = 128, kGramThreads = 256, kGramRow = kGramPix + 1;
constexpr int kGramAcc = (kGramMaxK * (kGramMaxK + 1) / 2 + kGramThreads - 1) / kGramThreads;

template <int BR, int BC>
__global__ void __launch_bounds__(kGramThreads)
    zernike_gram_kernel(const double* table, const double* params, int param_stride, int n, unsigned pitch,
                        unsigned item_stride, int nmax, int kdim, int K, const double* slots,
                        const double* fac, const double* pupil, double* partial) {
  extern __shared__ double zbuf[];
  const int item = blockIdx.y, tid = threadIdx.x;
  const double* p = params + (size_t)item * param_stride;
  const int npairs = K * (K + 1) / 2;
  double* out = partial + ((size_t)item * gridDim.x + blockIdx.x) * (npairs + 1);
  if (p[ZP_ENABLE] == 0.0) {
    for (int q = tid; q <= npairs; q += kGramThreads) out[q] = 0.0;
    return;
  }
  const double dx = p[ZP_DX], dy = p[ZP_DY], radius = p[ZP_RADIUS];
  const bool origin_y = p[ZP_ORIGIN_Y] != 0.0;
  const double co = p[ZP_COS_OFF], so = p[ZP_SIN_OFF];
  int pi[kGramAcc], pj[kGramAcc];
  double acc[kGramAcc];
#pragma unroll
  for (int a = 0; a < kGramAcc; ++a) {
    acc[a] = 0.0;
    int q = tid + a * kGramThreads, i = 0;
    if (q < npairs) {
      while (q >= K - i) { q -= K - i; ++i; }
      pi[a] = i; pj[a] = i + q;
    } else {
      pi[a] = pj[a] = -1;
    }
  }
  double count = 0.0;
  const size_t total = item_stride;
  for (size_t chunk = blockIdx.x; chunk * kGramPix < total; chunk += gridDim.x) {
    int valid = 0;
    if (tid < kGramPix) {
      const size_t m = chunk * kGramPix + tid;
      int r = 0, c = 0;
      double rr = 0.0, rho = 2.0, x = 0.0, y = 0.0;
      if (m < total && layout_unmap<BR, BC>(m, n, pitch, r, c)) {
        x = (double)(c - n / 2) * dx;
        y = (double)(r - n / 2) * dy;
        rr = sqrt(__dadd_rn(__dmul_rn(x, x), __dmul_rn(y, y)));
        rho = rr / radius;
        valid = rho <= 1.0 && (!pupil || pupil[(size_t)item * item_stride + m] != 0.0);
      }
      if (valid) {
        double c1 = 1.0, s1 = 0.0;
        if (rr > 0.0) {
          c1 = (origin_y ? y : x) / rr;
          s1 = (origin_y ? x : y) / rr;
        }
        const double cr = c1 * co - s1 * so, sr = s1 * co + c1 * so;
        const double xj = 1.0 - 2.0 * rho * rho;
        double rho_pow = 1.0, cm = 1.0, sm = 0.0;
        for (int am = 0; am <= nmax; ++am) {
          const int kmax = (nmax - am) / 2;
          double pkm1 = 0.0, pk = 1.0;
          for (int k = 0; k <= kmax; ++k) {
            if (k > 0) {
              const double* abc = table + ((size_t)am * kdim + k) * 3;
              const double pn = (abc[0] * xj + abc[1]) * pk - abc[2] * pkm1;
              pkm1 = pk;
              pk = pn;
            }
            const size_t ci = (size_t)am * kdim + k;
            const int jc = (int)slots[2 * ci], js = (int)slots[2 * ci + 1];
            const double base = rho_pow * pk;
            if (jc >= 0) zbuf[jc * kGramRow + tid] = fac[jc] * base * cm;
            if (js >= 0) zbuf[js * kGramRow + tid] = fac[js] * base * sm;
          }
          rho_pow *= rho;
          const double cn = cm * cr - sm * sr;
          sm = sm * cr + cm * sr;
          cm = cn;
        }
        count += 1.0;
      } else {
        for (int j = 0; j < K; ++j) zbuf[j * kGramRow + tid] = 0.0;
// ... 122 lines not shown
```

Before: 2254 wavefronts/s.

## Defer the start field write and fuse it into the Zernike phase kernel

The start-field write is now deferred: the aperture and stop parameters are saved as a pending start and, when the next Zernike call covers the single group with every item enabled, one fused kernel computes the aperture value and applies the phase in one pass. This avoids writing the field once and then reading and rewriting it. A norm2 request made while the start is still pending is computed analytically from the aperture instead of from the field. The cost is extra host bookkeeping: parameter arrays are kept on the host and re-pushed if the arena slab changes, and every other entry point has to settle the pending write, so a missed settle would break correctness.

```diff
diff --git a/include/paos_hip.h b/include/paos_hip.h
--- a/include/paos_hip.h
+++ b/include/paos_hip.h
@@ -99,6 +99,7 @@
                     int n_blocks);
 int paos_copy_yardstick(paos_ctx* ctx, int reps, double* ms_per_launch, double* bytes_per_launch);
 int paos_record_set_stats(paos_ctx* ctx, unsigned long long* found, unsigned long long* rendered);
+int paos_start_stats(paos_ctx* ctx, unsigned long long* fused, unsigned long long* written);
 int paos_ctx_set_pruning(paos_ctx* ctx, int on);
 int paos_run_passes_live(paos_ctx* ctx, const paos_pass* passes, int n_passes, const double* blocks,
                          int n_blocks, const double* live_rows);
diff --git a/paos_amd/_lib.py b/paos_amd/_lib.py
--- a/paos_amd/_lib.py
+++ b/paos_amd/_lib.py
@@ -76,6 +76,7 @@
     "paos_run_passes": (ctypes.c_int, [_c_ctx, ctypes.POINTER(Pass), ctypes.c_int, _dbl_p, ctypes.c_int]),
     "paos_copy_yardstick": (ctypes.c_int, [_c_ctx, ctypes.c_int, _dbl_p, _dbl_p]),
     "paos_record_set_stats": (ctypes.c_int, [_c_ctx, ctypes.POINTER(ctypes.c_ulonglong), ctypes.POINTER(ctypes.c_ulonglong)]),
+    "paos_start_stats": (ctypes.c_int, [_c_ctx, ctypes.POINTER(ctypes.c_ulonglong), ctypes.POINTER(ctypes.c_ulonglong)]),
     "paos_ctx_set_pruning": (ctypes.c_int, [_c_ctx, ctypes.c_int]),
     "paos_run_passes_live": (ctypes.c_int, [_c_ctx, ctypes.POINTER(Pass), ctypes.c_int, _dbl_p, ctypes.c_int, _dbl_p]),
     "paos_zernike": (ctypes.c_int, [_c_ctx, ctypes.c_int, ctypes.c_int, _dbl_p, _dbl_p, ctypes.c_int, _dbl_p]),
@@ -535,6 +536,11 @@
                     "paos_record_set_stats")
         return int(found.value), int(rendered.value)
 
+    def start_stats(self):
+        fused, written = ctypes.c_ulonglong(0), ctypes.c_ulonglong(0)
+        self._check(self._lib.paos_start_stats(self._ctx, ctypes.byref(fused), ctypes.byref(written)), "paos_start_stats")
+        return int(fused.value), int(written.value)
+
     def set_pruning(self, on):
         self._check(self._lib.paos_ctx_set_pruning(self._ctx, 1 if on else 0), "paos_ctx_set_pruning")
 
diff --git a/paos_amd/csrc/paos_hip.hip b/paos_amd/csrc/paos_hip.hip
--- a/paos_amd/csrc/paos_hip.hip
+++ b/paos_amd/csrc/paos_hip.hip
@@ -61,6 +61,7 @@
   hipEvent_t fence[kArenaSlabs] = {};
   bool fenced[kArenaSlabs] = {};
   bool used[kArenaSlabs] = {};
+  unsigned long long switches = 0;
 };
 
 }
@@ -75,6 +76,17 @@
   unsigned long long map_key = 0;
   std::vector<double> start_key;
   double* start_norm2 = nullptr;
+  struct PendingStart {
+    bool owed = false;
+    int shape = 0;
+    double re = 0.0, im = 0.0;
+    bool any_stop = false, one_group = false;
+    std::vector<double> aperture, flags, rows, cols, goff, glen, members;
+    const double *dp = nullptr, *ds = nullptr, *drows = nullptr, *dcols = nullptr, *dgoff = nullptr, *dglen = nullptr,
+                 *dmembers = nullptr;
+    unsigned long long switches_at = 0;
+  } start;
+  unsigned long long start_fused = 0, start_written = 0;
   cx<double>* psd_scratch = nullptr;
   int* psd_bad = nullptr;
   double* psf_partial = nullptr;
@@ -174,6 +186,7 @@
   a.used[next] = true;
   a.cur = next;
   a.head = 0;
+  ++a.switches;
   return PAOS_OK;
 }
 
@@ -193,6 +206,7 @@
     (void)hipHostFree(a.host);
     (void)hipFree(a.dev);
     a.host = h; a.dev = d; a.cap = cap; a.head = 0; a.cur = 0; a.left = -1;
+    a.switches += kArenaSlabs;
     for (int k = 0; k < kArenaSlabs; ++k) a.fenced[k] = a.used[k] = false;
     a.used[0] = true;
     return PAOS_OK;
@@ -770,8 +784,13 @@
   c->dyn_pending = false;
   return PAOS_OK;
 }
-#define SETTLE_SCALE(c) do { if (c) { (c)->norm2_of_field = false; if ((c)->dyn_pending) { int rc_ = settle_scale(c); if (rc_) return rc_; } } } while (0)
-#define DROP_SCALE(c) do { if (c) { (c)->norm2_of_field = false; if ((c)->dyn_pending) { int rc_ = settle_scale(c, true); if (rc_) return rc_; } } } while (0)
+int settle_start(paos_ctx* c);
+int start_write(paos_ctx* c, const double* norm2);
+int owed_start_blocks(paos_ctx* c);
+#define SETTLE_START(c) do { if ((c) && (c)->start.owed) { int rc_ = settle_start(c); if (rc_) return rc_; } } while (0)
+#define SETTLE_SCALE_KEEP_START(c) do { if (c) { (c)->norm2_of_field = false; if ((c)->dyn_pending) { int rc_ = settle_scale(c); if (rc_) return rc_; } } } while (0)
+#define SETTLE_SCALE(c) do { SETTLE_START(c); SETTLE_SCALE_KEEP_START(c); } while (0)
+#define DROP_SCALE(c) do { SETTLE_START(c); if (c) { (c)->norm2_of_field = false; if ((c)->dyn_pending) { int rc_ = settle_scale(c, true); if (rc_) return rc_; } } } while (0)
 
 
 bool frugal_sizes(const paos_ctx* c) {
@@ -1154,6 +1173,7 @@
 int run_passes_impl(paos_ctx* c, const paos_pass* passes, int n_passes, const double* blocks, int n_blocks,
                     const double* entry_rows, bool entry_stale, int* final_ticket, int final_mode, const double* entry_cols) {
   if (!c || !passes || !blocks || n_passes < 0 || n_blocks < 1) return fail(c, PAOS_EINVAL, "bad pass program");
+  SETTLE_START(c);
   c->norm2_of_field = false;
   if (final_ticket && c->norm_busy[next_norm_slot(c)])
     return fail(c, PAOS_EINVAL, "64 power reductions outstanding: fetch earlier tickets (paos_norm2_fetch) first");
@@ -1755,6 +1775,7 @@
   const double *dp = nullptr, *ds = nullptr, *dcompute = nullptr, *dpower_of = nullptr;
   int rc;
   if ((rc = arena_push(c, aperture, (size_t)c->batch * AP_STRIDE, &dp))) return rc;
+  const unsigned long long switches_at = c->arena.switches;
   if ((rc = arena_push(c, flags.data(), flags.size(), &ds))) return rc;
   if ((rc = arena_push(c, compute.data(), compute.size(), &dcompute))) return rc;
   if ((rc = arena_push(c, power_of.data(), power_of.size(), &dpower_of))) return rc;
@@ -1797,9 +1818,9 @@
   if ((rc = arena_push(c, members.data(), members.size(), &dmembers))) return rc;
   const dim3 block(kPwThreads);
   bool power_found = false;
+  static const bool memo = [] { const char* e = getenv("PAOS_START_POWER_MEMO"); return !(e && e[0] == '0'); }();
+  std::vector<double> key;
   if (any_stop) {
-    static const bool memo = [] { const char* e = getenv("PAOS_START_POWER_MEMO"); return !(e && e[0] == '0'); }();
-    std::vector<double> key;
     key.reserve(3 + (size_t)c->batch * (AP_STRIDE + 1));
     key.push_back((double)shape); key.push_back(re); key.push_back(im);
     key.insert(key.end(), aperture, aperture + (size_t)c->batch * AP_STRIDE);
@@ -1810,34 +1831,92 @@
       HIPCHK(c, hipMemcpyAsync(c->norm2, c->start_norm2, (size_t)c->batch * sizeof(double), hipMemcpyDeviceToDevice, c->stream));
     } else {
       c->start_key.clear();
+#define START_POWER(T, BRV, S)                                                                          \
+  do {                                                                                                  \
+    hipLaunchKernelGGL((start_power_kernel<T, BRV, Lay<T>::BC, S>), dim3(c->nparts, c->batch), block, 0, \
+                       c->stream, dp, c->n, c->pitch, c->item_stride, re, im, c->partial, dcompute);    \
+    hipLaunchKernelGGL(norm2_final_kernel, dim3(c->batch), block, 0, c->stream, c->partial, c->norm2,   \
+                       c->nparts, ds, 1, dpower_of);                                                    \
+  } while (0)
+      if (c->precision == PAOS_F64) {
+        if (shape == PAOS_SHAPE_ELLIPSE) START_POWER(double, BR, 0); else START_POWER(double, BR, 1);
+      } else {
+        if (shape == PAOS_SHAPE_ELLIPSE) F32_BR_SWITCH(c, START_POWER(float, FBR, 0)); else F32_BR_SWITCH(c, START_POWER(float, FBR, 1));
+      }
+#undef START_POWER
+      HIPCHK(c, hipGetLastError());
+      if (!c->start_norm2) HIPCHK(c, hipMalloc(&c->start_norm2, (size_t)c->batch * sizeof(double)));
+      HIPCHK(c, hipMemcpyAsync(c->start_norm2, c->norm2, (size_t)c->batch * sizeof(double), hipMemcpyDeviceToDevice, c->stream));
       if (memo) c->start_key = std::move(key);
     }
   }
-#define START_LAUNCH(T, BRV, S)                                                                         \
-  do {                                                                                                  \
-    if (any_stop && !power_found) {                                                                     \
-      hipLaunchKernelGGL((start_power_kernel<T, BRV, Lay<T>::BC, S>), dim3(c->nparts, c->batch), block, 0, \
-                         c->stream, dp, c->n, c->pitch, c->item_stride, re, im, c->partial, dcompute);  \
-      hipLaunchKernelGGL(norm2_final_kernel, dim3(c->batch), block, 0, c->stream, c->partial, c->norm2,   \
-                         c->nparts, ds, 1, dpower_of);                                                  \
-    }                                                                                                   \
-    hipLaunchKernelGGL((start_write_kernel<T, BRV, Lay<T>::BC, S>), dim3(pw_blocks(c), c->batch), block, 0, \
-                       c->stream, (cx<T>*)c->field, dp, c->n, c->pitch, c->item_stride, re, im,          \
-                       (const double*)c->norm2, ds, drows, dgoff, dglen, dmembers, dcols);              \
-  } while (0)
+  paos_ctx::PendingStart& st = c->start;
+  st.shape = shape; st.re = re; st.im = im; st.any_stop = any_stop;
+  st.one_group = c->batch > 0 && glen[0] == (double)c->batch;
+  st.dp = dp; st.ds = ds; st.drows = drows; st.dcols = dcols; st.dgoff = dgoff; st.dglen = dglen; st.dmembers = dmembers;
+  st.switches_at = switches_at;
+  const char* fuse_env = getenv("PAOS_FUSE_START");
+  const bool fuse = !(fuse_env && fuse_env[0] == '0');
+  if (fuse && drows && dcols) {
+    st.aperture.assign(aperture, aperture + (size_t)c->batch * AP_STRIDE);
+    st.flags = flags;
+    st.rows.assign(write_rows, write_rows + (size_t)2 * c->batch);
+    st.cols = rounded_cols(c, write_cols);
+    st.goff = goff; st.glen = glen; st.members = members;
+    st.owed = true;
+    return PAOS_OK;
+  }
+  return start_write(c, (const double*)c->norm2);
+}
+
+}
+
+namespace {
+
+int start_write(paos_ctx* c, const double* norm2) {
+  const paos_ctx::PendingStart& st = c->start;
+  const dim3 block(kPwThreads);
+#define START_WRITE(T, BRV, S)                                                                            \
+  hipLaunchKernelGGL((start_write_kernel<T, BRV, Lay<T>::BC, S>), dim3(pw_blocks(c), c->batch), block, 0, \
+                     c->stream, (cx<T>*)c->field, st.dp, c->n, c->pitch, c->item_stride, st.re, st.im,    \
+                     norm2, st.ds, st.drows, st.dgoff, st.dglen, st.dmembers, st.dcols)
   if (c->precision == PAOS_F64) {
-    if (shape == PAOS_SHAPE_ELLIPSE) START_LAUNCH(double, BR, 0); else START_LAUNCH(double, BR, 1);
+    if (st.shape == PAOS_SHAPE_ELLIPSE) START_WRITE(double, BR, 0); else START_WRITE(double, BR, 1);
   } else {
-    if (shape == PAOS_SHAPE_ELLIPSE) F32_BR_SWITCH(c, START_LAUNCH(float, FBR, 0)); else F32_BR_SWITCH(c, START_LAUNCH(float, FBR, 1));
-  }
-#undef START_LAUNCH
+    if (st.shape == PAOS_SHAPE_ELLIPSE) F32_BR_SWITCH(c, START_WRITE(float, FBR, 0)); else F32_BR_SWITCH(c, START_WRITE(float, FBR, 1));
+  }
+#undef START_WRITE
   HIPCHK(c, hipGetLastError());
-  if (any_stop && !power_found && !c->start_key.empty()) {
-    if (!c->start_norm2) HIPCHK(c, hipMalloc(&c->start_norm2, (size_t)c->batch * sizeof(double)));
-    HIPCHK(c, hipMemcpyAsync(c->start_norm2, c->norm2, (size_t)c->batch * sizeof(double), hipMemcpyDeviceToDevice, c->stream));
-  }
-  return PAOS_OK;
-}
+  ++c->start_written;
+  return PAOS_OK;
+}
+
+int owed_start_blocks(paos_ctx* c) {
+  paos_ctx::PendingStart& st = c->start;
+  if (c->arena.switches <= st.switches_at + 1) return PAOS_OK;
+  int rc;
+  if ((rc = arena_push(c, st.aperture.data(), st.aperture.size(), &st.dp))) return rc;
+  st.switches_at = c->arena.switches;
+  if ((rc = arena_push(c, st.flags.data(), st.flags.size(), &st.ds))) return rc;
+  if ((rc = arena_push(c, st.rows.data(), st.rows.size(), &st.drows))) return rc;
+  if ((rc = arena_push(c, st.cols.data(), st.cols.size(), &st.dcols))) return rc;
+  if ((rc = arena_push(c, st.goff.data(), st.goff.size(), &st.dgoff))) return rc;
+  if ((rc = arena_push(c, st.glen.data(), st.glen.size(), &st.dglen))) return rc;
+  if ((rc = arena_push(c, st.members.data(), st.members.size(), &st.dmembers))) return rc;
+  return PAOS_OK;
+}
+
+int settle_start(paos_ctx* c) {
+  (void)hipSetDevice(c->device);
+  c->start.owed = false;
+  int rc = owed_start_blocks(c);
+  if (rc) return rc;
+  return start_write(c, c->start_norm2);
+}
+
+}
+
+extern "C" {
 
 int paos_start(paos_ctx* c, double re, double im, int shape, const double* aperture, const double* stop) {
   DROP_SCALE(c);
@@ -2264,7 +2343,20 @@
     if ((rc = arena_push(c, same_as, (size_t)c->batch, &dsame))) return rc;
   }
   const dim3 grid(c->nparts, c->batch), block(kPwThreads);
-  if (c->precision == PAOS_F64)
+  if (c->start.owed) {
+    paos_ctx::PendingStart& st = c->start;
+    if ((rc = owed_start_blocks(c))) return rc;
+    const double* sn = c->start_norm2;
+#define SN_LAUNCH(T, BRV, S)                                                                                       \
+  hipLaunchKernelGGL((start_norm2_partial_kernel<T, BRV, Lay<T>::BC, S>), grid, block, 0, c->stream, st.dp, st.re, \
+                     st.im, sn, st.ds, c->partial, c->n, c->pitch, c->item_stride, dlead, drows, dcols)
+    if (c->precision == PAOS_F64) {
+      if (st.shape == PAOS_SHAPE_ELLIPSE) SN_LAUNCH(double, BR, 0); else SN_LAUNCH(double, BR, 1);
+    } else {
+      if (st.shape == PAOS_SHAPE_ELLIPSE) F32_BR_SWITCH(c, SN_LAUNCH(float, FBR, 0)); else F32_BR_SWITCH(c, SN_LAUNCH(float, FBR, 1));
+    }
+#undef SN_LAUNCH
+  } else if (c->precision == PAOS_F64)
     hipLaunchKernelGGL((norm2_partial_kernel<double, BR, Lay<double>::BC>), grid, block, 0, c->stream,
                        (const cx<double>*)c->field, c->partial, c->n, c->pitch, c->item_stride, dlead, 1, drows, dcols);
   else
@@ -2275,7 +2367,17 @@
 }
 
 int paos_norm2_enqueue_box(paos_ctx* c, const double* live_rows, const double* live_cols, const double* same_as, int* ticket) {
-  SETTLE_SCALE(c);
+  SETTLE_SCALE_KEEP_START(c);
+  if (c && c->start.owed) {
+    const paos_ctx::PendingStart& st = c->start;
+    bool same = live_rows && live_cols && check_rows(c, live_rows) == PAOS_OK && check_rows(c, live_cols) == PAOS_OK &&
+                !std::memcmp(live_rows, st.rows.data(), st.rows.size() * sizeof(double));
+    if (same) {
+      const std::vector<double> lc = rounded_cols(c, live_cols);
+      same = !std::memcmp(lc.data(), st.cols.data(), st.cols.size() * sizeof(double));
+    }
+    if (!same) SETTLE_START(c);
+  }
   if (c && live_cols) {
     int rc = check_rows(c, live_cols);
     if (rc) return rc;
@@ -2451,6 +2553,13 @@
   return PAOS_OK;
 }
 
+int paos_start_stats(paos_ctx* c, unsigned long long* fused, unsigned long long* written) {
+  if (!c || !fused || !written) return fail(c, PAOS_EINVAL, "bad start-stats request");
+  *fused = c->start_fused;
+  *written = c->start_written;
+  return PAOS_OK;
+}
+
 int paos_copy_yardstick(paos_ctx* c, int reps, double* ms_per_launch, double* bytes_per_launch) {
   SETTLE_SCALE(c);
   if (c) (void)hipSetDevice(c->device);
@@ -2522,6 +2631,12 @@
     for (int k = ZP_DX; k < param_stride; ++k)
       if (!std::isfinite(q[k])) return fail(c, PAOS_EINVAL, "non-finite Zernike parameter");
   }
+  bool fuse_start = false;
+  if (c->start.owed) {
+    fuse_start = c->start.one_group && !host_wfe && !use_pupil;
+    for (int i = 0; i < c->batch && fuse_start; ++i) fuse_start = params[(size_t)i * param_stride + ZP_ENABLE] != 0.0;
+    if (!fuse_start) { int rc_ = settle_start(c); if (rc_) return rc_; }
+  }
   const double *dt = nullptr, *dp = nullptr;
   int rc = arena_push(c, table, (size_t)(nmax + 1) * kdim * 3, &dt);
   if (rc) return rc;
@@ -2594,6 +2709,27 @@
       m_end = (unsigned)(hi / c->br) * c->pitch;
     }
   }
+  if (fuse_start) {
+    paos_ctx::PendingStart& st = c->start;
+    st.owed = false;
+    if ((rc = owed_start_blocks(c))) return rc;
+    const double* sn = c->start_norm2;
+#define SZ_LAUNCH(T, BRV, S, NC)                                                                                        \
+  hipLaunchKernelGGL((start_zernike_kernel<T, BRV, Lay<T>::BC, S, NC>), grid, block, 0, c->stream, (cx<T>*)c->field,    \
+                     st.dp, st.re, st.im, sn, st.ds, st.drows, st.dcols, dt, dp, param_stride, c->n, c->pitch,          \
+                     c->item_stride, nmax, kdim, m_first, m_end, dgoff, dglen, dmembers)
+#define SZ_SHAPE(T, BRV, NC) do { if (st.shape == PAOS_SHAPE_ELLIPSE) SZ_LAUNCH(T, BRV, 0, NC); else SZ_LAUNCH(T, BRV, 1, NC); } while (0)
+    if (c->precision == PAOS_F64) {
+      if (nmax <= 8) SZ_SHAPE(double, BR, 8); else SZ_SHAPE(double, BR, 0);
+    } else {
+      if (nmax <= 8) F32_BR_SWITCH(c, SZ_SHAPE(float, FBR, 8)); else F32_BR_SWITCH(c, SZ_SHAPE(float, FBR, 0));
+    }
+#undef SZ_SHAPE
+#undef SZ_LAUNCH
+    HIPCHK(c, hipGetLastError());
+    ++c->start_fused;
+    return PAOS_OK;
+  }
 #define ZK_LAUNCH(T, BRV, NC)                                                                                          \
   hipLaunchKernelGGL((zernike_kernel<T, BRV, Lay<T>::BC, NC>), grid, block, 0, c->stream, (cx<T>*)c->field, dt, dp,   \
                      param_stride, c->n, c->pitch, c->item_stride, nmax, kdim, wfe, pupil, m_first, m_end, dgoff, dglen, \
@@ -2611,14 +2747,14 @@
 
 int paos_zernike(paos_ctx* c, int nmax, int kdim, const double* table, const double* params,
                  int param_stride, double* host_wfe) {
-  SETTLE_SCALE(c);
+  SETTLE_SCALE_KEEP_START(c);
   if (c) (void)hipSetDevice(c->device);
   return zernike_apply(c, nmax, kdim, table, params, param_stride, host_wfe, false);
 }
 
 int paos_zernike_like(paos_ctx* c, int nmax, int kdim, const double* table, const double* params,
                       int param_stride, const double* same_as, double* host_wfe) {
-  SETTLE_SCALE(c);
+  SETTLE_SCALE_KEEP_START(c);
   if (c) (void)hipSetDevice(c->device);
   return zernike_apply(c, nmax, kdim, table, params, param_stride, host_wfe, false, same_as);
 }
diff --git a/paos_amd/csrc/pointwise.h b/paos_amd/csrc/pointwise.h
--- a/paos_amd/csrc/pointwise.h
+++ b/paos_amd/csrc/pointwise.h
@@ -570,6 +570,43 @@
   if (threadIdx.x == 0) partial[(size_t)item * gridDim.x + blockIdx.x] = s;
 }
 
+template <typename T, int SHAPE>
+__device__ __forceinline__ void start_value(const ApertureEval<SHAPE>& ap, bool on, bool scaled, double s, double v0re,
+                                            double v0im, int r, int c, double& x, double& y) {
+  const double w = on ? ap.weight(ap.mask(r, c)) : 1.0;
+  x = w == 1.0 ? v0re : (w == 0.0 ? 0.0 : (double)(T)__dmul_rn(v0re, w));
+  y = w == 1.0 ? v0im : (w == 0.0 ? 0.0 : (double)(T)__dmul_rn(v0im, w));
+  if (scaled) { x = __dmul_rn(x, s); y = __dmul_rn(y, s); }
+}
+
+struct StartWindow {
+  size_t first, total, work;
+  unsigned in_lo, span;
+  bool boxed;
+  template <int BR, int BC>
+  __device__ __forceinline__ void init(const double* rows, const double* cols, int item, int n, unsigned pitch,
+                                       unsigned item_stride) {
+    total = item_stride; first = 0;
+    if (rows) {
+      first = (size_t)((int)rows[2 * item] / BR) * pitch;
+      total = (size_t)(((int)rows[2 * item + 1] + BR - 1) / BR) * pitch;
+      if (total > item_stride) total = item_stride;
+    }
+    in_lo = 0; span = pitch; boxed = cols != nullptr;
+    if (cols) {
+      in_lo = (unsigned)((int)cols[2 * item] / BC) * (BR * BC);
+      unsigned h = (unsigned)(((int)cols[2 * item + 1] + BC - 1) / BC) * (BR * BC);
+      if (h > (unsigned)n * BR) h = (unsigned)n * BR;
+      span = h > in_lo ? h - in_lo : 0;
+    }
+    const size_t nbr = (total - first) / pitch;
+    work = boxed ? nbr * span : total - first;
+  }
+  __device__ __forceinline__ size_t at(size_t j, unsigned pitch) const {
+    return boxed ? first + (j / span) * pitch + in_lo + (j % span) : first + j;
+  }
+};
+
 template <typename T, int BR, int BC, int SHAPE>
 __global__ void start_write_kernel(cx<T>* field, const double* params, int n, unsigned pitch,
                                    unsigned item_stride, double vre, double vim, const double* norm2,
@@ -586,31 +623,13 @@
   const bool scaled = stop[item] != 0.0;
   const double s = scaled ? 1.0 / sqrt(norm2[item]) : 1.0;
   const double v0re = (double)(T)vre, v0im = (double)(T)vim;
-  size_t total = item_stride, first = 0;
-  if (rows) {
-    first = (size_t)((int)rows[2 * item] / BR) * pitch;
-    total = (size_t)(((int)rows[2 * item + 1] + BR - 1) / BR) * pitch;
-    if (total > item_stride) total = item_stride;
-  }
-  unsigned in_lo = 0, span = pitch;
-  if (cols) {
-    in_lo = (unsigned)((int)cols[2 * item] / BC) * (BR * BC);
-    unsigned h = (unsigned)(((int)cols[2 * item + 1] + BC - 1) / BC) * (BR * BC);
-    if (h > (unsigned)n * BR) h = (unsigned)n * BR;
-    span = h > in_lo ? h - in_lo : 0;
-  }
-  const size_t nbr = (total - first) / pitch;
-  const size_t work = cols ? nbr * span : total - first;
-  for (size_t j = (size_t)blockIdx.x * blockDim.x + threadIdx.x; j < work; j += (size_t)gridDim.x * blockDim.x) {
-    const size_t m = cols ? first + (j / span) * pitch + in_lo + (j % span) : first + j;
+  StartWindow win;
+  win.init<BR, BC>(rows, cols, item, n, pitch, item_stride);
+  for (size_t j = (size_t)blockIdx.x * blockDim.x + threadIdx.x; j < win.work; j += (size_t)gridDim.x * blockDim.x) {
+    const size_t m = win.at(j, pitch);
     int r, c;
     double x = 0.0, y = 0.0;
-    if (layout_unmap<BR, BC>(m, n, pitch, r, c)) {
-      const double w = on ? ap.weight(ap.mask(r, c)) : 1.0;
-      x = w == 1.0 ? v0re : (w == 0.0 ? 0.0 : (double)(T)__dmul_rn(v0re, w));
-      y = w == 1.0 ? v0im : (w == 0.0 ? 0.0 : (double)(T)__dmul_rn(v0im, w));
-      if (scaled) { x = __dmul_rn(x, s); y = __dmul_rn(y, s); }
-    }
+    if (layout_unmap<BR, BC>(m, n, pitch, r, c)) start_value<T, SHAPE>(ap, on, scaled, s, v0re, v0im, r, c, x, y);
     for (int g = 0; g < glen; ++g) field[(size_t)(int)members[g] * item_stride + m] = {(T)x, (T)y};
   }
 }
@@ -989,6 +1008,109 @@
 
 enum : int { ZP_ENABLE = 0, ZP_DX, ZP_DY, ZP_RADIUS, ZP_ORIGIN_Y, ZP_COS_OFF, ZP_SIN_OFF, ZP_INV_WL, ZP_HEAD };
 
+template <int NMAXC>
+__device__ __forceinline__ double zernike_wfe(double x, double y, double rr, double rho, bool origin_y, double co, double so,
+                                              const double* table, const double* coef_c, const double* coef_s, int nmax,
+                                              int kdim) {
+  double wfe = 0.0;
+  double c1 = 1.0, s1 = 0.0;
+  if (rr > 0.0) {
+    c1 = (origin_y ? y : x) / rr;
+    s1 = (origin_y ? x : y) / rr;
+  }
+  const double cr = c1 * co - s1 * so, sr = s1 * co + c1 * so;
+  const double xj = 1.0 - 2.0 * rho * rho;
+  double rho_pow = 1.0, cm = 1.0, sm = 0.0;
+  auto order = [&](int am, int k_end) __attribute__((always_inline)) {
+    double pkm1 = 0.0, pk = 1.0;
+    for (int k = 0; k <= k_end; ++k) {
+      if (k > 0) {
+        const double* abc = table + ((size_t)am * kdim + k) * 3;
+        const double pn = (abc[0] * xj + abc[1]) * pk - abc[2] * pkm1;
+        pkm1 = pk;
+        pk = pn;
+      }
+      const size_t ci = (size_t)am * kdim + k;
+      wfe += (rho_pow * pk) * (coef_c[ci] * cm + coef_s[ci] * sm);
+    }
+    rho_pow *= rho;
+    const double cn = cm * cr - sm * sr;
+    sm = sm * cr + cm * sr;
+    cm = cn;
+  };
+  if constexpr (NMAXC > 0) {
+#pragma unroll
+    for (int am = 0; am <= NMAXC; ++am) {
+      if (am > nmax) break;
+      const int kmax = (nmax - am) / 2;
+      double pkm1 = 0.0, pk = 1.0;
+#pragma unroll
+      for (int k = 0; k <= (NMAXC - am) / 2; ++k) {
+        if (k > kmax) break;
+        if (k > 0) {
+          const double* abc = table + ((size_t)am * kdim + k) * 3;
+          const double pn = (abc[0] * xj + abc[1]) * pk - abc[2] * pkm1;
+          pkm1 = pk;
+          pk = pn;
+        }
+        const size_t ci = (size_t)am * kdim + k;
+        wfe += (rho_pow * pk) * (coef_c[ci] * cm + coef_s[ci] * sm);
+      }
+      rho_pow *= rho;
+      const double cn = cm * cr - sm * sr;
+      sm = sm * cr + cm * sr;
+      cm = cn;
+    }
+  } else {
+    for (int am = 0; am <= nmax; ++am) order(am, (nmax - am) / 2);
+  }
+  return wfe;
+}
+
+template <typename T>
+__device__ __forceinline__ void zernike_members(cx<T>* field, const double* params, int param_stride, unsigned item_stride,
+                                                const double* members, int glen, size_t m, double wfe, bool twins,
+                                                cx<double> lead) {
+  const double turns = __dmul_rn(6.283185307179586, wfe);
+  constexpr int kZernikeGroup = 8;
+  int g = 0;
+  for (; g + kZernikeGroup <= glen; g += kZernikeGroup) {
+    cx<T>* f4[kZernikeGroup];
+    cx<double> v4[kZernikeGroup];
+    double iw[kZernikeGroup];
+#pragma unroll
+    for (int q = 0; q < kZernikeGroup; ++q) {
+      const int it = (int)members[g + q];
+      f4[q] = field + (size_t)it * item_stride + m;
+      iw[q] = params[(size_t)it * param_stride + ZP_INV_WL];
+    }
+    if (twins) {
+#pragma unroll
+      for (int q = 0; q < kZernikeGroup; ++q) v4[q] = lead;
+    } else {
+#pragma unroll
+      for (int q = 0; q < kZernikeGroup; ++q) v4[q] = {(double)f4[q]->x, (double)f4[q]->y};
+    }
+#pragma unroll
+    for (int q = 0; q < kZernikeGroup; ++q) {
+      double sn, cs;
+      sincos_fast(__dmul_rn(turns, iw[q]), &sn, &cs);
+      *f4[q] = {(T)__dsub_rn(__dmul_rn(v4[q].x, cs), __dmul_rn(v4[q].y, sn)),
+                (T)__dadd_rn(__dmul_rn(v4[q].x, sn), __dmul_rn(v4[q].y, cs))};
+    }
+  }
+  for (; g < glen; ++g) {
+    const int it = (int)members[g];
+    const double arg = __dmul_rn(turns, params[(size_t)it * param_stride + ZP_INV_WL]);
+    double sn, cs;
+    sincos_fast(arg, &sn, &cs);
+    cx<T>* f = field + (size_t)it * item_stride;
+    const cx<double> v = twins ? lead : cx<double>{(double)f[m].x, (double)f[m].y};
+    f[m] = {(T)__dsub_rn(__dmul_rn(v.x, cs), __dmul_rn(v.y, sn)),
+            (T)__dadd_rn(__dmul_rn(v.x, sn), __dmul_rn(v.y, cs))};
+  }
+}
+
 template <typename T, int BR, int BC, int NMAXC = 0>
 __global__ void zernike_kernel(cx<T>* field, const double* table, const double* params,
                                int param_stride, int n, unsigned pitch, unsigned item_stride,
@@ -1017,100 +1139,104 @@
     const bool masked = rho > 1.0 || (pupil && pupil[(size_t)item * item_stride + m] == 0.0);
     double wfe = 0.0;
     if (!masked) {
-      double c1 = 1.0, s1 = 0.0;
-      if (rr > 0.0) {
-        c1 = (origin_y ? y : x) / rr;
-        s1 = (origin_y ? x : y) / rr;
-      }
-      const double cr = c1 * co - s1 * so, sr = s1 * co + c1 * so;
-      const double xj = 1.0 - 2.0 * rho * rho;
-      double rho_pow = 1.0, cm = 1.0, sm = 0.0;
-      auto order = [&](int am, int k_end) __attribute__((always_inline)) {
-        double pkm1 = 0.0, pk = 1.0;
-        for (int k = 0; k <= k_end; ++k) {
-          if (k > 0) {
-            const double* abc = table + ((size_t)am * kdim + k) * 3;
-            const double pn = (abc[0] * xj + abc[1]) * pk - abc[2] * pkm1;
-            pkm1 = pk;
-            pk = pn;
-          }
-          const size_t ci = (size_t)am * kdim + k;
-          wfe += (rho_pow * pk) * (coef_c[ci] * cm + coef_s[ci] * sm);
-        }
-        rho_pow *= rho;
-        const double cn = cm * cr - sm * sr;
-        sm = sm * cr + cm * sr;
-        cm = cn;
-      };
-      if constexpr (NMAXC > 0) {
-#pragma unroll
-        for (int am = 0; am <= NMAXC; ++am) {
-          if (am > nmax) break;
-          const int kmax = (nmax - am) / 2;
-          double pkm1 = 0.0, pk = 1.0;
-#pragma unroll
-          for (int k = 0; k <= (NMAXC - am) / 2; ++k) {
-            if (k > kmax) break;
-            if (k > 0) {
-              const double* abc = table + ((size_t)am * kdim + k) * 3;
-              const double pn = (abc[0] * xj + abc[1]) * pk - abc[2] * pkm1;
-              pkm1 = pk;
-              pk = pn;
-            }
-            const size_t ci = (size_t)am * kdim + k;
-            wfe += (rho_pow * pk) * (coef_c[ci] * cm + coef_s[ci] * sm);
-          }
-          rho_pow *= rho;
-          const double cn = cm * cr - sm * sr;
-          sm = sm * cr + cm * sr;
-          cm = cn;
-        }
-      } else {
-        for (int am = 0; am <= nmax; ++am) order(am, (nmax - am) / 2);
-      }
-      const double turns = __dmul_rn(6.283185307179586, wfe);
-      constexpr int kZernikeGroup = 8;
+      wfe = zernike_wfe<NMAXC>(x, y, rr, rho, origin_y, co, so, table, coef_c, coef_s, nmax, kdim);
       cx<double> lead = {0.0, 0.0};
       if (twins) { const cx<T>* fl = field + (size_t)item * item_stride + m; lead = {(double)fl->x, (double)fl->y}; }
-      int g = 0;
-      for (; g + kZernikeGroup <= glen; g += kZernikeGroup) {
-        cx<T>* f4[kZernikeGroup];
-        cx<double> v4[kZernikeGroup];
-        double iw[kZernikeGroup];
-#pragma unroll
-        for (int q = 0; q < kZernikeGroup; ++q) {
-          const int it = (int)members[g + q];
-          f4[q] = field + (size_t)it * item_stride + m;
-          iw[q] = params[(size_t)it * param_stride + ZP_INV_WL];
+      zernike_members<T>(field, params, param_stride, item_stride, members, glen, m, wfe, twins, lead);
+    }
+    if (wfe_out && item == 0) wfe_out[(size_t)r * n + c] = masked ? __longlong_as_double(0x7ff8000000000000LL) : wfe;
+  }
+}
+
+template <typename T, int BR, int BC, int SHAPE, int NMAXC = 0>
+__global__ void start_zernike_kernel(cx<T>* field, const double* ap_params, double vre, double vim, const double* norm2,
+                                     const double* stop, const double* rows, const double* cols, const double* table,
+                                     const double* params, int param_stride, int n, unsigned pitch, unsigned item_stride,
+                                     int nmax, int kdim, unsigned m_first, unsigned m_end, const double* grp_off,
+                                     const double* grp_len, const double* grp_members) {
+  const int item = blockIdx.y;
+  const int glen = (int)grp_len[item];
+  if (glen == 0) return;
+  const double* members = grp_members + (int)grp_off[item];
+  const double* ap_p = ap_params + (size_t)item * AP_STRIDE;
+  ApertureEval<SHAPE> ap;
+  ap.init(ap_p, ap_p + AP_THETA);
+  const bool on = ap_p[AP_ENABLE] != 0.0;
+  const bool scaled = stop[item] != 0.0;
+  const double s = scaled ? 1.0 / sqrt(norm2[item]) : 1.0;
+  const double v0re = (double)(T)vre, v0im = (double)(T)vim;
+  const double* p = params + (size_t)item * param_stride;
+  const double dx = p[ZP_DX], dy = p[ZP_DY], radius = p[ZP_RADIUS];
+  const bool origin_y = p[ZP_ORIGIN_Y] != 0.0;
+  const double co = p[ZP_COS_OFF], so = p[ZP_SIN_OFF];
+  const double* coef_c = p + ZP_HEAD;
+  const double* coef_s = coef_c + (size_t)(nmax + 1) * kdim;
+  const size_t z_end = m_end < item_stride ? m_end : item_stride;
+  StartWindow win;
+  win.init<BR, BC>(rows, cols, item, n, pitch, item_stride);
+  for (size_t j = (size_t)blockIdx.x * blockDim.x + threadIdx.x; j < win.work; j += (size_t)gridDim.x * blockDim.x) {
+    const size_t m = win.at(j, pitch);
+    int r, c;
+    double sx = 0.0, sy = 0.0;
+    bool phased = false;
+    if (layout_unmap<BR, BC>(m, n, pitch, r, c)) {
+      start_value<T, SHAPE>(ap, on, scaled, s, v0re, v0im, r, c, sx, sy);
+      if (m >= m_first && m < z_end) {
+        const double x = (double)(c - n / 2) * dx, y = (double)(r - n / 2) * dy;
+        const double rr = sqrt(__dadd_rn(__dmul_rn(x, x), __dmul_rn(y, y)));
+        const double rho = rr / radius;
+        if (!(rho > 1.0)) {
+          const double wfe = zernike_wfe<NMAXC>(x, y, rr, rho, origin_y, co, so, table, coef_c, coef_s, nmax, kdim);
+          zernike_members<T>(field, params, param_stride, item_stride, members, glen, m, wfe, true,
+                             cx<double>{(double)(T)sx, (double)(T)sy});
+          phased = true;
         }
-        if (twins) {
-#pragma unroll
-          for (int q = 0; q < kZernikeGroup; ++q) v4[q] = lead;
-        } else {
-#pragma unroll
-          for (int q = 0; q < kZernikeGroup; ++q) v4[q] = {(double)f4[q]->x, (double)f4[q]->y};
-        }
-#pragma unroll
-        for (int q = 0; q < kZernikeGroup; ++q) {
-          double sn, cs;
-          sincos_fast(__dmul_rn(turns, iw[q]), &sn, &cs);
-          *f4[q] = {(T)__dsub_rn(__dmul_rn(v4[q].x, cs), __dmul_rn(v4[q].y, sn)),
-                    (T)__dadd_rn(__dmul_rn(v4[q].x, sn), __dmul_rn(v4[q].y, cs))};
-        }
-      }
-      for (; g < glen; ++g) {
-        const int it = (int)members[g];
-        const double arg = __dmul_rn(turns, params[(size_t)it * param_stride + ZP_INV_WL]);
-        double sn, cs;
-        sincos_fast(arg, &sn, &cs);
-        cx<T>* f = field + (size_t)it * item_stride;
-        const cx<double> v = twins ? lead : cx<double>{(double)f[m].x, (double)f[m].y};
-        f[m] = {(T)__dsub_rn(__dmul_rn(v.x, cs), __dmul_rn(v.y, sn)),
-                (T)__dadd_rn(__dmul_rn(v.x, sn), __dmul_rn(v.y, cs))};
-      }
-    }
-    if (wfe_out && item == 0) wfe_out[(size_t)r * n + c] = masked ? __longlong_as_double(0x7ff8000000000000LL) : wfe;
-  }
+      }
+    }
+    if (!phased)
+      for (int g = 0; g < glen; ++g) field[(size_t)(int)members[g] * item_stride + m] = {(T)sx, (T)sy};
+  }
+}
+
+template <typename T, int BR, int BC, int SHAPE>
+__global__ void start_norm2_partial_kernel(const double* ap_params, double vre, double vim, const double* norm2,
+                                           const double* stop, double* partial, int n, unsigned pitch,
+                                           unsigned item_stride, const double* enable, const double* rows,
+                                           const double* cols) {
+  const int item = blockIdx.y;
+  if (enable && enable[item] == 0.0) return;
+  __shared__ double sh[kPwThreads / 64];
+  const double* ap_p = ap_params + (size_t)item * AP_STRIDE;
+  ApertureEval<SHAPE> ap;
+  ap.init(ap_p, ap_p + AP_THETA);
+  const bool on = ap_p[AP_ENABLE] != 0.0;
+  const bool scaled = stop[item] != 0.0;
+  const double s = scaled ? 1.0 / sqrt(norm2[item]) : 1.0;
+  const double v0re = (double)(T)vre, v0im = (double)(T)vim;
+  size_t first = (size_t)((int)rows[2 * item] / BR) * pitch;
+  size_t total = (size_t)(((int)rows[2 * item + 1] + BR - 1) / BR) * pitch;
+  if (total > item_stride) total = item_stride;
+  double acc = 0.0;
+  const size_t step = (size_t)gridDim.x * blockDim.x;
+  size_t m = (size_t)blockIdx.x * blockDim.x + threadIdx.x;
+  if (m < first) m += (first - m + step - 1) / step * step;
+  unsigned in_lo = 0, in_hi = (unsigned)n * BR;
+  if (cols) {
+    in_lo = (unsigned)((int)cols[2 * item] / BC) * (BR * BC);
+    const unsigned h = (unsigned)(((int)cols[2 * item + 1] + BC - 1) / BC) * (BR * BC);
+    in_hi = h < in_hi ? h : in_hi;
+  }
+  for (; m < total; m += step) {
+    const unsigned off = (unsigned)(m % pitch);
+    if (off >= in_hi || off < in_lo) continue;
+    int r, c;
+    double sx = 0.0, sy = 0.0;
+    if (layout_unmap<BR, BC>(m, n, pitch, r, c)) start_value<T, SHAPE>(ap, on, scaled, s, v0re, v0im, r, c, sx, sy);
+    const double x = (double)(T)sx, y = (double)(T)sy;
+    acc += __dadd_rn(__dmul_rn(x, x), __dmul_rn(y, y));
+  }
+  const double sum = block_sum(acc, sh);
+  if (threadIdx.x == 0) partial[(size_t)item * gridDim.x + blockIdx.x] = sum;
 }
 
 constexpr int kGramMaxK = 64, kGramPix = 128, kGramThreads = 256, kGramRow = kGramPix + 1;
```

Result: no change. 2272 wavefronts/s, median of 6 (+0.8%).
